# JosefAlbers/Phi-3-Vision-MLX

Measured on AMD Instinct MI355X. Metric: decode tokens/sec through generate()'s loop (reference-defined; bare graph replays: device_rate) + prefill ms, Phi-3-Vision bf16 1-image VQA, higher is better.
Workload: dtype bf16; 1 GPU; Phi-3-Vision single 336x336 image VQA (BASELINE configs[1]); 17 crops, 2509 image tokens + 22 text tokens, prompt 2531, B=1 per GPU, greedy, EOS suppressed; parallelism=batch-sharded replicas x1, batch_per_gpu=1, tiny=False

## Files before the change

### include/p3v.h

```cpp
#ifndef P3V_H
#define P3V_H
#include <stdint.h>

#ifdef __cplusplus
extern "C" {
#endif

#define P3V_VERSION 600
#define P3V_OK 0
#define P3V_ERR_ARG (-22)
#define P3V_ERR_LAUNCH (-5)
#define P3V_ERR_UNSUPPORTED (-95)
#define P3V_ERR_HIP (-14)

typedef struct {
  int cu_count, lds_per_cu, wave_size, clock_khz, mem_clock_khz, mem_bus_bits;
  int64_t hbm_bytes;
  char arch[32];
} p3v_props_t;

int p3v_version(void);
int p3v_device_props(int device, p3v_props_t* out );
const char* p3v_strerror(int code);

// ... 50 lines not shown
int p3v_gemv(const p3v_gemv_args_t* args , void* stream);

typedef struct {
  const uint16_t* x; const uint8_t* W; const float* w_scale; void* out;
  const uint16_t* resid; const uint16_t* norm_w;
  float norm_eps;
  int M, N, K;
  int epilogue;
} p3v_gemv_fp8_args_t;
int p3v_gemv_fp8(const p3v_gemv_fp8_args_t* args , void* stream);
int p3v_dequant_fp8(const uint8_t* w8, const float* w_scale, uint16_t* out_bf16, int rows, int K, void* stream);

int p3v_pack_b13(const uint16_t* W, int rows, int K, int silu_pairs, void* out, int32_t* info, void* stream);
int p3v_unpack_b13(const void* packed, int rows, int K, int silu_pairs, int exp_base, uint16_t* out_bf16, void* stream);
typedef struct {
  const uint16_t* x; const void* W; void* out;
  const uint16_t* resid; const uint16_t* norm_w;
  float norm_eps;
  int M, N, K;
  int epilogue;
  int exp_base, silu_pairs;
} p3v_gemv_b13_args_t;
int p3v_gemv_b13(const p3v_gemv_b13_args_t* args , void* stream);
int p3v_gemv_b13_plan(int N, int K, int epilogue, int n_cu, int* out );

typedef struct {
  const uint8_t* A; const float* a_scale; const uint8_t* W; const float* w_scale;
  uint16_t* out; const uint16_t* resid;
  int M, N, K, lda, ldw, ldo, epilogue;
} p3v_gemm_fp8_args_t;
int p3v_gemm_fp8(const p3v_gemm_fp8_args_t* args , void* stream);
int p3v_quant_fp8_rows(const uint16_t* x, const uint16_t* norm_w , float eps, uint8_t* q, float* scale,
                       int rows, int K, void* stream);

int p3v_rope_table(const float* pos, const float* inv_freq, float scale, float* cos_out, float* sin_out,
                   int n_pos, int half_dim, void* stream);

int p3v_rope_kv_append(const uint16_t* qkv, const float* cos_t, const float* sin_t,
                       uint16_t* q_out, uint16_t* k_dst, uint16_t* v_dst,
                       int B, int L, int n_heads, int n_kv, int hd,
                       int past, const int32_t* d_past, int dst_t, int dst_off_is_past,
                       int tab_t, int tab_div, float q_scale, void* stream);

int p3v_gemm_resid_norm(const p3v_gemm_args_t* gemm , const uint16_t* norm_w, float eps, uint16_t* normed, void* stream);

typedef struct {
  const float* cos_t; const float* sin_t;
  uint16_t* q_out; uint16_t* k_dst; uint16_t* v_dst;
  int B, L, n_heads, n_kv, hd;
  int past, dst_t, dst_off_is_past, tab_t, tab_div;
  float q_scale;
} p3v_qkv_split_t;
int p3v_gemm_qkv(const p3v_gemm_args_t* gemm , const p3v_qkv_split_t* split , void* stream);

typedef struct {
  const uint16_t* q;
  const uint16_t* k_past; const uint16_t* v_past;
  const uint16_t* k_new;  const uint16_t* v_new;
  uint16_t* out;
  const int32_t* pad_len;
  const int32_t* d_past;
  float* ws;
  int B, L, n_heads, n_kv, hd;
  int past, past_t, past_div, new_t, pad_div;
  int causal;
  float scale;
  int n_split;
  int new_is_cache;
  int q_prescaled;
} p3v_attn_args_t;
int p3v_attention(const p3v_attn_args_t* args , void* stream);
int64_t p3v_attention_ws_bytes(int B, int L, int n_heads, int hd, int n_split);
#define P3V_DECODE_MAX_L 16

typedef struct {
  const uint16_t* qkv; const float* cos_t; const float* sin_t;
  uint16_t* k_cache; uint16_t* v_cache; uint16_t* out;
  const int32_t* pad_len; const int32_t* d_past; float* ws;
  int B, L, n_heads, n_kv, hd, past, cache_t, rope_bstride, n_split;
  float scale;
  int merge_in_launch;
  const void* o_proj_w; uint16_t* o_proj_x; uint16_t* o_rearm; int o_n;
  const uint32_t* o_proj_sb;
} p3v_attn_decode_args_t;
int p3v_attention_decode(const p3v_attn_decode_args_t* args , void* stream);
int p3v_attention_decode_can_fuse_oproj(int B, int L, int n_heads, int hd, int n_split, int cache_t, int o_n, int merge_in_launch);
int p3v_attention_decode_fused_role(int wg, int n_heads, int n_split, int o_n, int map, int* out4);
#define P3V_FAMILY_MAX 16
#define P3V_FAMILY_INTS (2 + P3V_FAMILY_MAX)
int p3v_attention_decode_family(const p3v_attn_decode_args_t* args , const int32_t* family ,
                                const int32_t* family_host , void* stream);
int p3v_stage_rope(const float* cos_t, const float* sin_t, int past, const int32_t* d_past,
                   float* cos_out, float* sin_out, int B, int L, int tab_t, int half_dim, void* stream);

int p3v_kv_quantize(const uint16_t* k, const uint16_t* vt, uint8_t* k8, uint8_t* v8t, float* k_scale, float* v_scale,
                    int BH, int hd, int src_t, int dst_t, int t0, int n_tok, void* stream);
int p3v_kv_dequantize(const uint8_t* k8, const uint8_t* v8t, const float* k_scale, const float* v_scale, uint16_t* k,
                      uint16_t* vt, int BH, int hd, int src_t, int dst_t, int n_tok, void* stream);

int p3v_kv_quantize_mlx4(uint16_t* k, uint16_t* vt, uint32_t* k4, uint32_t* v4, float* k_sb, float* v_sb, int BH, int hd,
                         int cache_t, int n_tok, const uint16_t* qkv, const float* cos_t, const float* sin_t, int n_heads, int n_kv,
                         int past, int tab_t, int tab_div, void* stream);

typedef struct {
  const uint16_t* qkv; const float* cos_t; const float* sin_t;
  uint8_t* k8; uint8_t* v8t; float* k_scale; float* v_scale; uint16_t* out;
  const int32_t* pad_len; const int32_t* d_past; float* ws;
  int B, L, n_heads, n_kv, hd, past, cache_t, rope_bstride, n_split;
  float scale;
  int merge_in_launch;
  const uint8_t* o_proj_w8; const float* o_proj_scale; uint16_t* o_proj_x; uint16_t* o_rearm; int o_n;
} p3v_attn_decode_q8_args_t;
int p3v_attention_decode_q8(const p3v_attn_decode_q8_args_t* args , void* stream);
int p3v_attention_decode_q8_can_fuse_oproj(int B, int L, int n_heads, int hd, int n_split, int cache_t, int o_n, int merge_in_launch);

int p3v_im2col_patches(const float* pix, uint16_t* patches, int n_img, int img, int patch, int kpad, void* stream);
int p3v_clip_cls_rows(float* x, const uint16_t* cls, const uint16_t* pos, int n_img, int tokens, int dim, void* stream);

int p3v_hd_merge(const float* feats, const uint16_t* sub_gn, const uint16_t* glb_gn, uint16_t* out,
                 int h_crops, int w_crops, int grid , int C, void* stream);

int p3v_argmax(const uint16_t* logits, int32_t* out, int rows, int n, int64_t row_stride, void* stream);
int p3v_log_softmax(const uint16_t* x, uint16_t* y, int rows, int n, void* stream);
int p3v_topk(const uint16_t* x, int32_t* idx_out, int rows, int n, int k, int64_t row_stride, void* stream);

typedef struct {
  const uint16_t* x; const uint32_t* W; const uint32_t* sb; void* out;
  const uint16_t* resid; const uint16_t* norm_w; float norm_eps;
  int M, N, K;
  int epilogue;
} p3v_gemv_q4_args_t;
int p3v_gemv_q4(const p3v_gemv_q4_args_t* args , void* stream);
int p3v_dequant_q4(const uint32_t* w4, const uint32_t* sb, uint16_t* out_bf16, int rows, int K, void* stream);

int p3v_resample_u8(const uint8_t* in, uint8_t* out, int outer, int in_len, int out_len, int inner,
                    const int32_t* coeffs, const int32_t* bounds, int ksize, void* stream);
int p3v_hd_preprocess(const uint8_t* resized, int rh, int rw, int top, int hp, int portrait, const double* lut,
                      const float* hw, const int32_t* hi, const float* ww, const int32_t* wi, float* pixel_values,
                      int n_slots, void* stream);

int p3v_lora_down(const uint16_t* x, const float* lora_a, float* t, int M, int K, int r, void* stream);
int p3v_lora_up(const uint16_t* y, const float* t, const float* lora_b, float scale, int epilogue,
                const uint16_t* resid, uint16_t* out, int M, int N, int r, void* stream);

#define P3V_LORA_SLICE_K 256
typedef struct {
  const float* lora_a;
  const float* lora_b;
  int32_t rank;
  float scale;
} p3v_lora_entry_t;
int p3v_lora_rows_slices(int K);
int p3v_lora_down_rows(const uint16_t* x, const uint16_t* norm_w , float eps, const p3v_lora_entry_t* table,
                       const int32_t* row_adapter, float* t, int M, int K, int r_max, int n_slots, void* stream);
int p3v_lora_up_rows(const uint16_t* y, const float* t, const p3v_lora_entry_t* table, const int32_t* row_adapter,
                     int epilogue, const uint16_t* resid, uint16_t* out, int M, int N, int K, int r_max, int n_slots,
                     void* stream);

int p3v_add_i32(int32_t* x, int n, int delta, void* stream);
int p3v_store_token(const int32_t* tok, int32_t* history, const int32_t* d_step, int32_t* tok_next,
                    int B, int max_steps, void* stream);
int p3v_step_begin(const int32_t* tok, const uint16_t* table, uint16_t* x_out, const float* cos_t, const float* sin_t,
                   const int32_t* d_past, float* cos_out, float* sin_out, int B, int hidden, int vocab, int tab_t,
                   int half_dim, int32_t* zero_buf ,
                   int n_zero, void* stream);
int p3v_step_end(const uint16_t* logits, int32_t* next_tok, int32_t* tok, int32_t* history, int32_t* d_step,
// ... 115 lines not shown
```

### phi-3-vision-mlx_amd/_lib.py

```python
import ctypes as C
import os

_HERE = os.path.dirname(os.path.abspath(__file__))
LIB_PATH = os.environ.get("P3V_LIB") or os.path.join(_HERE, "libp3v.so")

P3V_OK = 0
(EPI_NONE, EPI_BIAS, EPI_BIAS_QGELU, EPI_BIAS_GELU, EPI_BIAS_RESID_F32, EPI_RESID_BF16, EPI_SILU_MUL, EPI_PATCH,
 EPI_F32) = range(9)
DECODE_MAX_L = 16

vp, i32, i64, f32 = C.c_void_p, C.c_int, C.c_int64, C.c_float


class Props(C.Structure):
    _fields_ = [("cu_count", i32), ("lds_per_cu", i32), ("wave_size", i32), ("clock_khz", i32),
                ("mem_clock_khz", i32), ("mem_bus_bits", i32), ("hbm_bytes", i64), ("arch", C.c_char * 32)]


class GemmArgs(C.Structure):
    _fields_ = [("A", vp), ("W", vp), ("out", vp), ("bias", vp), ("resid", vp), ("pos", vp),
                ("M", i32), ("N", i32), ("K", i32), ("lda", i32), ("ldw", i32), ("ldo", i32),
                ("epilogue", i32), ("patches_per_img", i32), ("ws", vp), ("ws_bytes", i64)]


class QkvSplit(C.Structure):
    _fields_ = [("cos_t", vp), ("sin_t", vp), ("q_out", vp), ("k_dst", vp), ("v_dst", vp),
                ("B", i32), ("L", i32), ("n_heads", i32), ("n_kv", i32), ("hd", i32),
                ("past", i32), ("dst_t", i32), ("dst_off_is_past", i32), ("tab_t", i32), ("tab_div", i32), ("q_scale", f32)]


class GemvArgs(C.Structure):
    _fields_ = [("x", vp), ("W", vp), ("out", vp), ("resid", vp), ("norm_w", vp), ("norm_eps", f32),
                ("M", i32), ("N", i32), ("K", i32), ("epilogue", i32)]


class GemvStep(C.Structure):
    _fields_ = [("tok", vp), ("embed_table", vp), ("vocab", i32), ("x_out", vp),
                ("cos_t", vp), ("sin_t", vp), ("cos_out", vp), ("sin_out", vp), ("tab_t", i32), ("half_dim", i32),
                ("next_tok", vp), ("tok_out", vp), ("history", vp), ("d_step", vp), ("ticket", vp), ("amax_ws", vp), ("max_steps", i32),
                ("d_past", vp)]


GEMV_STEP_WS_BYTES = 1024 * 8 + 9 * 128


class GemvF8Args(C.Structure):
    _fields_ = [("x", vp), ("W", vp), ("w_scale", vp), ("out", vp), ("resid", vp), ("norm_w", vp), ("norm_eps", f32),
                ("M", i32), ("N", i32), ("K", i32), ("epilogue", i32)]


class GemvB13Args(C.Structure):
    _fields_ = [("x", vp), ("W", vp), ("out", vp), ("resid", vp), ("norm_w", vp), ("norm_eps", f32),
                ("M", i32), ("N", i32), ("K", i32), ("epilogue", i32), ("exp_base", i32), ("silu_pairs", i32)]


class GemmF8Args(C.Structure):
    _fields_ = [("A", vp), ("a_scale", vp), ("W", vp), ("w_scale", vp), ("out", vp), ("resid", vp),
                ("M", i32), ("N", i32), ("K", i32), ("lda", i32), ("ldw", i32), ("ldo", i32), ("epilogue", i32)]


class AttnArgs(C.Structure):
    _fields_ = [("q", vp), ("k_past", vp), ("v_past", vp), ("k_new", vp), ("v_new", vp), ("out", vp),
                ("pad_len", vp), ("d_past", vp), ("ws", vp),
                ("B", i32), ("L", i32), ("n_heads", i32), ("n_kv", i32), ("hd", i32),
                ("past", i32), ("past_t", i32), ("past_div", i32), ("new_t", i32), ("pad_div", i32),
                ("causal", i32), ("scale", f32), ("n_split", i32), ("new_is_cache", i32), ("q_prescaled", i32)]


class GemvQ4Args(C.Structure):
    _fields_ = [("x", vp), ("W", vp), ("sb", vp), ("out", vp), ("resid", vp), ("norm_w", vp), ("norm_eps", f32),
                ("M", i32), ("N", i32), ("K", i32), ("epilogue", i32)]


class AttnDecArgs(C.Structure):
    _fields_ = [("qkv", vp), ("cos_t", vp), ("sin_t", vp), ("k_cache", vp), ("v_cache", vp), ("out", vp),
                ("pad_len", vp), ("d_past", vp), ("ws", vp),
                ("B", i32), ("L", i32), ("n_heads", i32), ("n_kv", i32), ("hd", i32), ("past", i32),
                ("cache_t", i32), ("rope_bstride", i32), ("n_split", i32), ("scale", f32), ("merge_in_launch", i32),
                ("o_proj_w", vp), ("o_proj_x", vp), ("o_rearm", vp), ("o_n", i32),
                ("o_proj_sb", vp)]


class AttnDecQ8Args(C.Structure):
    _fields_ = [("qkv", vp), ("cos_t", vp), ("sin_t", vp), ("k8", vp), ("v8t", vp), ("k_scale", vp), ("v_scale", vp),
                ("out", vp), ("pad_len", vp), ("d_past", vp), ("ws", vp),
                ("B", i32), ("L", i32), ("n_heads", i32), ("n_kv", i32), ("hd", i32), ("past", i32),
                ("cache_t", i32), ("rope_bstride", i32), ("n_split", i32), ("scale", f32), ("merge_in_launch", i32),
                ("o_proj_w8", vp), ("o_proj_scale", vp), ("o_proj_x", vp), ("o_rearm", vp), ("o_n", i32)]


class SampleRow(C.Structure):
    _fields_ = [("temperature", f32), ("top_k", i32), ("top_p", f32), ("seed_lo", C.c_uint32), ("seed_hi", C.c_uint32),
                ("counter", i32)]


LOGPROBS_MAX = 8


class LogprobRecord(C.Structure):
    _fields_ = [("token", C.c_int32), ("logprob", f32), ("rank", C.c_int32), ("n_top", C.c_int32),
                ("top_id", C.c_int32 * LOGPROBS_MAX), ("top_logprob", f32 * LOGPROBS_MAX)]


LOGPROB_WORDS = C.sizeof(LogprobRecord) // 4


class PenaltyRow(C.Structure):
    _fields_ = [("repetition", f32), ("frequency", f32), ("presence", f32), ("flags", C.c_int32)]


PENALTY_WORDS = C.sizeof(PenaltyRow) // 4
PENALTY_ACTIVE, PENALTY_BIAS = 1, 2


class GuideRow(C.Structure):
    _fields_ = [("flags", C.c_int32), ("n_states", C.c_int32), ("state", C.c_int32), ("reserved", C.c_int32)]


GUIDE_WORDS = C.sizeof(GuideRow) // 4
GUIDE_MAX_STATES, GUIDE_ACTIVE, GUIDE_DONE = 255, 1, -1


class KvCopyJob(C.Structure):
    _fields_ = [("k_src", vp), ("v_src", vp), ("k_dst", vp), ("v_dst", vp),
                ("ks_src", vp), ("vs_src", vp), ("ks_dst", vp), ("vs_dst", vp),
                ("B_src", i32), ("b_src", i32), ("T_src", i32), ("t0_src", i32),
                ("B_dst", i32), ("b_dst", i32), ("T_dst", i32), ("t0_dst", i32), ("n_tok", i32)]


KV_FORK_MAX_DST = 15
FAMILY_MAX, FAMILY_INTS = 16, 18


class KvFork(C.Structure):
    _fields_ = [("k_src", vp), ("v_src", vp), ("k_dst", vp), ("v_dst", vp),
                ("ks_src", vp), ("vs_src", vp), ("ks_dst", vp), ("vs_dst", vp),
                ("B_src", i32), ("b_src", i32), ("T_src", i32), ("t0_src", i32),
                ("B_dst", i32), ("T_dst", i32), ("t0_dst", i32), ("n_tok", i32), ("n_dst", i32),
                ("b_dst", i32 * KV_FORK_MAX_DST)]


class SpecState(C.Structure):
    _fields_ = [("tok", vp), ("ctx", vp), ("ctl", vp), ("amax", vp), ("ticket", vp),
                ("history", vp), ("rec", vp), ("d_step", vp), ("d_past", vp),
                ("ctx_cap", i32), ("hist_cap", i32), ("rec_cap", i32), ("n_max", i32), ("n_min", i32)]


SPEC_REC_INTS, SPEC_CTL_INTS, SPEC_NGRAM_CAP = 18, 8, 8
SPEC_CTL_N, SPEC_CTL_NDRAFT, SPEC_CTL_FORCED, SPEC_CTL_REPLAY, SPEC_CTL_NLIMIT, SPEC_CTL_ACC = range(6)
KV_COPY_MAX_JOBS = 4
LORA_SLICE_K, LORA_MAX_RANK = 256, 64
SAMPLE_MAX_N, SAMPLE_MAX_ROWS = 32768, 1024
SIGNATURES = {
    "p3v_version": (i32, []),
    "p3v_device_props": (i32, [i32, C.POINTER(Props)]),
    "p3v_strerror": (C.c_char_p, [i32]),
    "p3v_set_tuning": (i32, [C.c_char_p, i32]),
    "p3v_get_tuning": (i32, [C.c_char_p, C.POINTER(i32)]),
    "p3v_embed_gather": (i32, [vp, vp, vp, i32, i32, i32, vp]),
    "p3v_rmsnorm": (i32, [vp, vp, vp, i32, i32, f32, vp]),
    "p3v_layernorm": (i32, [vp, vp, vp, vp, i32, i32, i32, f32, vp]),
    "p3v_gemm": (i32, [C.POINTER(GemmArgs), vp]),
    "p3v_gemm_ws_bytes": (i64, [i32, i32, i32, i32]),
# ... 98 lines not shown
```

### phi-3-vision-mlx_amd/csrc/p3v_attention.hip

```cpp
#include <stdlib.h>

#include "p3v_common.h"
#include "p3v_attn_shared.h"
#include "p3v_dot_bf16.h"
#include "p3v_dot_f8.h"
#include "p3v_dot_q4.h"

struct AttnP {
  const bf16_t* q; const bf16_t* k_past; const bf16_t* v_past; const bf16_t* k_new; const bf16_t* v_new;
  bf16_t* out; const int32_t* pad_len; const int32_t* d_past; float* ws;
  int B, L, nh, nkv, past, past_t, past_div, new_t, pad_div, causal, split_mode, n_split, new_is_cache;
  float scale;
  int head_group;
  float sc2;
  int q_prescaled;
};

template <int HD>
__global__ void __launch_bounds__(256) k_attn(AttnP p) {
  constexpr int KSTR = HD * 2 + 16;
  constexpr int VSTR = 64 * 2 + 16;
  constexpr int NKS = HD / 32;
  constexpr int NDT = HD / 16;
  constexpr int CPR = HD / 8;
  __shared__ __attribute__((aligned(16))) unsigned char Ks[64 * KSTR];
  __shared__ __attribute__((aligned(16))) unsigned char Vt[HD * VSTR];

  const int tid = threadIdx.x, lane = tid & 63, wave = tid >> 6;
  const int g = lane >> 4, qi = lane & 15;
  const int b = blockIdx.z, head = blockIdx.y, kvh = head / (p.nh / p.nkv);
  const int past = p.d_past ? *p.d_past : p.past;
  const int total = past + p.L;
  const int pad = p.pad_len ? p.pad_len[b / p.pad_div] : 0;
  const float sc2 = p.sc2;

  int q0, kv_begin, kv_end;
  bool active;
  if (p.split_mode) {
    q0 = 0;
    const int chunk = ((total + p.n_split - 1) / p.n_split + 63) & ~63;
    kv_begin = blockIdx.x * chunk;
    kv_end = min(total, kv_begin + chunk);
    active = wave == 0;
  } else {
    q0 = blockIdx.x * 64 + wave * 16;
    kv_begin = 0;
    kv_end = p.causal ? min(total, past + blockIdx.x * 64 + 64) : total;
    active = q0 < p.L;
  }
  if (pad > kv_begin) kv_begin = pad & ~63;

  const int qrow = q0 + qi;
  const bool qvalid = qrow < p.L;
  bf16x8_t qf[NKS];
  {
    const bf16_t* qp = p.q + (((size_t)b * p.nh + head) * p.L + (qvalid ? qrow : 0)) * HD + 8 * g;
#pragma unroll
    for (int ks = 0; ks < NKS; ++ks) {
      u32x4_t v = *(const u32x4_t*)(qp + 32 * ks);
      if (!qvalid) v = (u32x4_t){0, 0, 0, 0};
      qf[ks] = __builtin_bit_cast(bf16x8_t, v);
    }
  }
  const int qpos = past + qrow;

  const bf16_t* kp_base = p.k_past + ((size_t)(b / p.past_div) * p.nkv + kvh) * (size_t)p.past_t * HD;
  const bf16_t* vp_base = p.v_past + ((size_t)(b / p.past_div) * p.nkv + kvh) * (size_t)HD * p.past_t;
  const bf16_t* kn_base = p.k_new + ((size_t)b * p.nkv + kvh) * (size_t)p.new_t * HD;
  const bf16_t* vn_base = p.v_new + ((size_t)b * p.nkv + kvh) * (size_t)HD * p.new_t;

  float m_run = -INFINITY, l_run = 0.f;
  f32x4_t o[NDT];
#pragma unroll
  for (int d = 0; d < NDT; ++d) o[d] = (f32x4_t){0.f, 0.f, 0.f, 0.f};

  for (int kv0 = kv_begin; kv0 < kv_end; kv0 += 64) {
    __syncthreads();
    for (int i = tid; i < 64 * CPR; i += 256) {
      const int key = i / CPR, c = i % CPR, t = kv0 + key;
      u32x4_t kv = {0, 0, 0, 0};
      if (t < kv_end) {
        const bool from_past = t < past || p.new_is_cache;
        const bf16_t* ks = from_past ? kp_base + (size_t)t * HD : kn_base + (size_t)(t - past) * HD;
        kv = *(const u32x4_t*)(ks + c * 8);
      }
      *(u32x4_t*)(Ks + key * KSTR + c * 16) = kv;
    }
    for (int i = tid; i < HD * 8; i += 256) {
      const int d = i >> 3, c = i & 7, t0 = kv0 + c * 8;
// ... 1414 lines not shown
    const float m_use = m_new == -INFINITY ? 0.f : m_new;
    float l_t = 0.f;
#pragma unroll
    for (int r = 0; r < 4; ++r) {
      s[r] = __builtin_amdgcn_exp2f(s[r] - m_use);
      l_t += s[r];
    }
    l_run = rows_sum(l_t);
    m_run = m_new;
    DBG_T(5);
    const u32x2_t pw = {pack_bf16x2(s[0], s[1]), pack_bf16x2(s[2], s[3])};
    const s16x4_t pf = __builtin_bit_cast(s16x4_t, pw);
#pragma unroll
    for (int d = 0; d < NDT; ++d) {
      const s16x4_t vf = *(const s16x4_t*)(vtile + v_rd + d * 16 * 128);
      o[d] = __builtin_amdgcn_mfma_f32_16x16x16bf16_1k(vf, pf, o[d], 0, 0, 0);
    }
    DBG_T(6);
  }

  asm volatile("s_waitcnt vmcnt(0) lgkmcnt(0)" ::: "memory");
  __syncthreads();
  if (qvalid) {
    float* Ow = (float*)wreg + qi * HD;
#pragma unroll
    for (int d = 0; d < NDT; ++d) *(f32x4_t*)(Ow + 16 * d + 4 * g) = o[d];
    if (g == 0) { Ml[wave][qi][0] = m_run; Ml[wave][qi][1] = l_run; }
  }
  __syncthreads();
#pragma unroll 1
  for (int idx = tid; idx < n_vnew; idx += 256) {
    const int q = idx / HD, d = idx - q * HD;
    float mk[4], M = -INFINITY;
#pragma unroll
    for (int k = 0; k < 4; ++k) { mk[k] = Ml[k][q][0]; M = fmaxf(M, mk[k]); }
    const float Mu = M == -INFINITY ? 0.f : M;
    float acc = 0.f, lsum = 0.f;
#pragma unroll
    for (int k = 0; k < 4; ++k) {
      const float c = __builtin_amdgcn_exp2f(mk[k] - Mu);
      acc += c * ((const float*)(KV + k * WREG))[q * HD + d];
      lsum += c * Ml[k][q][1];
    }
    float* w = p.ws + ((((size_t)b * p.nh + head) * p.n_split + bx) * 16 + q) * (HD + 2);
    st_wt(w + d, acc);
    if (d == 0) { st_wt(w + HD, M); st_wt(w + HD + 1, lsum); }
  }
  DBG_T(7);
  DBG_W(13, false);
  if (p.merge && bx == p.n_split - 1) {
    __shared__ float merge_scratch[SPLIT_MERGE_SCRATCH(256)];
    split_merge<256>(p.ws + ((size_t)b * p.nh + head) * p.n_split * 16 * (HD + 2), p.out + (size_t)b * p.L * (p.nh * HD) + head * HD,
                     (size_t)p.nh * HD, p.L, p.n_split, nullptr, merge_scratch);
  }
  DBG_W(11, false);
}

struct FoMap { int bx, by, o_unit, o_unit2; };
__host__ __device__ __forceinline__ bool fo_map_ok(int n_split, int nh, int o_n) { return nh == 32 && o_n == 3072 && n_split >= 13 && n_split * nh <= 768; }
__host__ __device__ __forceinline__ FoMap fo_map(int L, int n_split, int nh, int n_units, bool two_on_last) {
  const int G = n_split * nh, base = G >> 8, r = G & 255;
  const int v = L & 255, slot = L >> 8, ns = base + (v < r ? 1 : 0);
  const int m0 = (base - 1) * 256 + 224;
  FoMap m;
  m.o_unit = m.o_unit2 = -1;
  if (L >= m0 && L < m0 + 32) { m.by = L - m0; m.bx = n_split - 1; return m; }
  const int before = L - m0 < 0 ? 0 : (L - m0 > 32 ? 32 : L - m0);
  const int u = L - before;
  m.by = u / (n_split - 1);
  m.bx = u - m.by * (n_split - 1);
  if (v < 224) {
    const int from_last = ns - 1 - slot;
    const int idx = base >= 2 || two_on_last ? (v >= r ? v - r : (224 - r) + v) : v;
    const int second = 224 + idx < n_units ? 224 + idx : -1;
    if (from_last == 0) { m.o_unit = v; if (two_on_last) m.o_unit2 = second; }
    else if (from_last == 1 && !two_on_last) m.o_unit = second;
  }
  return m;
}

#ifndef P3V_FO_SLEEP
#define P3V_FO_SLEEP 4
#endif
enum { FO_NONE = 0, FO_BF16 = 1, FO_F8 = 2, FO_Q4 = 3 };
struct FoP { const void* o_w; const void* o_scale; bf16_t* o_x; const bf16_t* out; int nh; };
template <int KIND, int NU = 1>
__device__ __forceinline__ void fo_project(const FoP f, const int o_wl, unsigned char* lds, const int o_wl2 = -1) {
  constexpr bool F8 = KIND == FO_F8, Q4 = KIND == FO_Q4;
  constexpr int HD = 96, NJ = KIND == FO_BF16 ? 6 : 3;
  const int tid = threadIdx.x, lane = tid & 63, wave = __builtin_amdgcn_readfirstlane(tid >> 6);
  const int Kd = f.nh * HD;
  const size_t row_bytes = (size_t)Kd * (Q4 ? 1 : F8 ? 2 : 4) / 2;
  const bool two = NU > 1 && o_wl2 >= 0;
  int o_u[NU];
  u32x4_t ow[NU][2][Q4 ? 1 : NJ];
  u32x2_t oq[NU][2][Q4 ? 3 : 1];
  uint32_t osb[NU][2][Q4 ? 3 : 1];
  uint32_t ores[NU];
  float osc[NU][2];
#pragma unroll
  for (int k = 0; k < NU; ++k) {
    o_u[k] = (k == 0 ? o_wl : o_wl2) * 4 + wave;
    if (k == 1 && !two) continue;
    const unsigned char* r0p = (const unsigned char*)f.o_w + (size_t)(2 * o_u[k]) * row_bytes;
    if (Q4) {
      const uint32_t* s0 = (const uint32_t*)f.o_scale + (size_t)(2 * o_u[k]) * (Kd / 64) + (lane >> 2);
#pragma unroll
      for (int j = 0; j < 3; ++j) {
        oq[k][0][j] = __builtin_nontemporal_load((const u32x2_t*)r0p + j * 64 + lane);
        oq[k][1][j] = __builtin_nontemporal_load((const u32x2_t*)(r0p + row_bytes) + j * 64 + lane);
        osb[k][0][j] = s0[j * 16];
        osb[k][1][j] = s0[Kd / 64 + j * 16];
      }
    } else {
#pragma unroll
      for (int j = 0; j < NJ; ++j) {
        ow[k][0][j] = __builtin_nontemporal_load((const u32x4_t*)r0p + j * 64 + lane);
        ow[k][1][j] = __builtin_nontemporal_load((const u32x4_t*)(r0p + row_bytes) + j * 64 + lane);
      }
    }
    ores[k] = *(const uint32_t*)(f.o_x + 2 * o_u[k]);
    osc[k][0] = F8 ? ((const float*)f.o_scale)[2 * o_u[k]] : 1.f;
    osc[k][1] = F8 ? ((const float*)f.o_scale)[2 * o_u[k] + 1] : 1.f;
  }
  {
    __shared__ int o_timeout;
    const uint32_t* src = (const uint32_t*)f.out;
    if (wave == 0) {
      bool to = false;
      const long long t_wait = wall_clock64();
      for (unsigned tries = 0;; ++tries) {
        const uint32_t c = lane < f.nh ? __hip_atomic_load(src + lane * (HD / 2) + HD / 2 - 1, __ATOMIC_RELAXED, __HIP_MEMORY_SCOPE_AGENT) : 0u;
        if (!__any((c & 0xffffu) == 0xffffu || (c >> 16) == 0xffffu)) break;
        if ((tries & 15u) == 15u && wall_clock64() - t_wait > 500000) { to = true; break; }
        __builtin_amdgcn_s_sleep(P3V_FO_SLEEP);
      }
      if (lane == 0) o_timeout = to;
    }
    TMARK(12);
    __syncthreads();
    uint32_t* xs = (uint32_t*)lds;
    bool timeout = o_timeout != 0;
    {
      const int NW = f.nh * HD / 2 / 4;
      uint32_t xv[6];
      for (unsigned tries = 0; !timeout; ++tries) {
        bool bad = false;
#pragma unroll
        for (int j = 0; j < 6; ++j) xv[j] = __hip_atomic_load(src + wave * NW + j * 64 + lane, __ATOMIC_RELAXED, __HIP_MEMORY_SCOPE_AGENT);
#pragma unroll
        for (int j = 0; j < 6; ++j) bad |= (xv[j] & 0xffffu) == 0xffffu || (xv[j] >> 16) == 0xffffu;
        if (!__any(bad)) break;
        if (tries >= (1u << 12)) timeout = true;
        __builtin_amdgcn_s_sleep(2);
      }
#pragma unroll
      for (int j = 0; j < 6; ++j) xs[wave * NW + j * 64 + lane] = xv[j];
      if (timeout && lane == 0) o_timeout = 1;
    }
    __syncthreads();
    timeout = o_timeout != 0;
    float* xsum = (float*)(lds + 6144);
    if (Q4) {
      if (tid < 192) {
        const u32x4_t a = ((const u32x4_t*)xs)[2 * tid], b = ((const u32x4_t*)xs)[2 * tid + 1];
        float t = 0.f;
#pragma unroll
        for (int j = 0; j < 4; ++j) t += (bf16lo(a[j]) + bf16hi(a[j])) + (bf16lo(b[j]) + bf16hi(b[j]));
        xsum[tid] = t;
      }
      __syncthreads();
    }
#pragma unroll
    for (int k = 0; k < NU; ++k) {
      if (k == 1 && !two) continue;
      float a0 = 0.f, a1 = 0.f;
      if (Q4) {
#pragma unroll
        for (int j = 0; j < 3; ++j) {
          const int pc = j * 64 + lane;
          const u32x4_t xa = ((const u32x4_t*)xs)[2 * pc], xb = ((const u32x4_t*)xs)[2 * pc + 1];
          const float X = xsum[pc], X128 = 128.f * X;
#pragma unroll
          for (int h = 0; h < 2; ++h) {
            const float D = dot8_q4(oq[k][h][j][1], xb, dot8_q4(oq[k][h][j][0], xa, 0.f));
            const float c = bf16lo(osb[k][h][j]) * (D - X128) + bf16hi(osb[k][h][j]) * X;
            if (h == 0) a0 += c; else a1 += c;
          }
        }
        if (k == 0) TMARK(13);
        a0 = wave_sum(a0);
        a1 = wave_sum(a1);
      } else if (F8) {
#pragma unroll
        for (int j = 0; j < 3; ++j) {
          const u32x4_t xa = ((const u32x4_t*)xs)[2 * (j * 64 + lane)], xb = ((const u32x4_t*)xs)[2 * (j * 64 + lane) + 1];
          a0 = dot16_f8(ow[k][0][j], xa, xb, a0);
          a1 = dot16_f8(ow[k][1][j], xa, xb, a1);
        }
        if (k == 0) TMARK(13);
        a0 = wave_sum(a0) * osc[k][0];
        a1 = wave_sum(a1) * osc[k][1];
      } else {
#pragma unroll
        for (int j = 0; j < 6; ++j) {
          const u32x4_t xa = ((const u32x4_t*)xs)[j * 64 + lane];
          a0 = dot8(ow[k][0][j], xa, a0);
          a1 = dot8(ow[k][1][j], xa, a1);
        }
        if (k == 0) TMARK(13);
        a0 = wave_sum(a0);
        a1 = wave_sum(a1);
      }
      if (lane == 0) {
        const float v0 = bf16lo(ores[k]) + bf16_round(a0), v1 = bf16hi(ores[k]) + bf16_round(a1);
        *(uint32_t*)(f.o_x + 2 * o_u[k]) = timeout ? 0x7fc07fc0u : pack_bf16x2(v0, v1);
      }
    }
    TMARK(14);
  }
}

template <int FO = 0>
__device__ __forceinline__ void attn_decode_body128(const AttnDecP& p, const int bx, const int by, const int bz, unsigned char* KV,
                                                    const int o_unit = -2, const int o_unit2 = -1) {
  constexpr int TK = 128, WK = 32, HD = 96, KROW = HD * 2, VROWB = TK * 2, NKS = 3, NDT = 6, CPR = 12;
  constexpr int KS_BYTES = WK * KROW;
  static_assert(KS_BYTES >= 16 * HD * 4, "a wave's O partial reuses its K slice");
  __shared__ __attribute__((aligned(16))) unsigned char Qs[16 * KROW];
  __shared__ float Ml[4][16][2];
  const int tid = threadIdx.x, lane = tid & 63, g = lane >> 4, qi = lane & 15;
  const int wave = __builtin_amdgcn_readfirstlane(tid >> 6);
  const int b = bz, head = by, kvh = (head * p.grp_magic) >> 16;
  const bool kv_writer = head == kvh * p.grp;
  unsigned char* kslice = KV + wave * KS_BYTES;
  unsigned char* vtile = KV + 4 * KS_BYTES;

  TMARK(0);
#ifdef P3V_ATTN_TIMING
  {
    unsigned hw, xcc;
    asm volatile("s_getreg_b32 %0, hwreg(HW_REG_HW_ID)" : "=s"(hw));
    asm volatile("s_getreg_b32 %0, hwreg(HW_REG_XCC_ID)" : "=s"(xcc));
    TVAL(15, (long long)(((xcc & 15) << 8) | (((hw >> 13) & 7) << 5) | (((hw >> 12) & 1) << 4) | ((hw >> 8) & 15)));
  }
#endif
  int past = p.past, pad = 0;
  const int past_lb = p.past;
  if (p.d_past) asm volatile("s_load_dword %0, %1, 0x0" : "=s"(past) : "s"(p.d_past) : "memory");
  if (p.pad_len) asm volatile("s_load_dword %0, %1, 0x0" : "=s"(pad) : "s"(p.pad_len + b) : "memory");

  const unsigned char* kc = (const unsigned char*)(p.k_cache + ((size_t)b * p.nkv + kvh) * (size_t)p.cache_t * HD);
  bf16_t* vc = p.v_cache + ((size_t)b * p.nkv + kvh) * (size_t)HD * p.cache_t;
  const int kv_lo = bx * TK, kv_hi = min(p.cache_t, kv_lo + TK);
  const size_t vrow = (size_t)p.cache_t * 2;
  auto issue_dma = [&]() {
    const int kv0 = min(kv_lo, p.cache_t - TK);
    const unsigned char* ksrc = kc + (size_t)(kv0 + WK * wave) * KROW;
    const unsigned char* vs = (const unsigned char*)vc + (size_t)kv0 * 2;
    const __amdgpu_buffer_rsrc_t rs_k = __builtin_amdgcn_make_buffer_rsrc((void*)ksrc, 0, 0xffffffff, 0x00020000);
    const __amdgpu_buffer_rsrc_t rs_v = __builtin_amdgcn_make_buffer_rsrc((void*)vs, 0, 0xffffffff, 0x00020000);
#pragma unroll
    for (int j = 0; j < 6; ++j) {
      const int i = j * 64 + lane, r0 = i / CPR, pc = i - r0 * CPR;
      const unsigned koff = r0 * KROW + ((pc ^ ((r0 >> 2) & 3)) << 4);
      __builtin_amdgcn_raw_ptr_buffer_load_lds(rs_k, (dec_lptr_t)(kslice + j * 1024), 16, koff, 0, 0, P3V_ATTN_AUX);
    }
#pragma unroll
    for (int j = 0; j < 6; ++j) {
      const int d = 24 * wave + 4 * j + (lane >> 4);
      const unsigned voff = (unsigned)d * (unsigned)vrow + ((((unsigned)lane & 15) ^ ((unsigned)d & 15)) << 4);
      __builtin_amdgcn_raw_ptr_buffer_load_lds(rs_v, (dec_lptr_t)(vtile + wave * 6144 + j * 1024), 16, voff, 0, 0, P3V_ATTN_AUX);
    }
  };

  const int row_w = (p.nh + 2 * p.nkv) * HD;
  const float* cos_b = p.cos_t + (size_t)b * p.rope_bstride * (HD / 2);
  const float* sin_b = p.sin_t + (size_t)b * p.rope_bstride * (HD / 2);
  const int tr = tid / CPR, tc = tid - tr * CPR;
  const bool rtask = tr < p.L;
  RopeRaw qraw, kraw;
  if (rtask) {
    const bf16_t* row = p.qkv + ((size_t)b * p.L + tr) * row_w;
    qraw = rope_fetch(row + head * HD, tc, cos_b + tr * (HD / 2), sin_b + tr * (HD / 2));
    const bf16_t* krow = row + (p.nh + kvh) * HD;
    kraw = qraw;
    kraw.x0 = *(const u32x4_t*)(krow + tc * 8);
    kraw.x1 = *(const u32x4_t*)(krow + (tc < 6 ? tc * 8 + 48 : tc * 8 - 48));
  }
  const bf16_t* vnew = p.qkv + (size_t)b * p.L * row_w + (p.nh + p.nkv + kvh) * HD;
  const int n_vnew = p.L * HD;
  bf16_t v_early = 0;
  if (tid < n_vnew) {
    const int r = tid / HD;
    v_early = vnew[(size_t)r * row_w + (tid - r * HD)];
  }
  const bool surely_live = p.d_past ? (past_lb < 0 || bx * TK < past_lb) : bx * TK < past_lb + p.L;
  if (surely_live) issue_dma();
  TMARK(7);
  const unsigned qs_lds = (unsigned)(size_t)(dec_lptr_t)Qs;
  if (tid < 16 * CPR) {
    u32x4_t v = {0, 0, 0, 0};
    if (rtask) v = rope_apply(qraw, tc);
    asm volatile("ds_write_b128 %0, %1" ::"v"(qs_lds + tr * KROW + ((tc ^ ((tr >> 2) & 3)) << 4)), "v"(v) : "memory");
  }

  asm volatile("s_waitcnt lgkmcnt(0)" : "+s"(past), "+s"(pad)::"memory");
  const int total = past + p.L;
// ... 90 lines not shown
        const int t = kv0 + WK * wave + 16 * kb + 4 * g + r;
        const bool vis = t < kv_end && t >= pad && t <= qpos && qpos >= pad;
        s[kb][r] = vis ? s[kb][r] * sc2 : -INFINITY;
        m_t = fmaxf(m_t, s[kb][r]);
      }
    m_t = rows_max(m_t);
    const float m_use = m_t == -INFINITY ? 0.f : m_t;
    float l_t = 0.f;
#pragma unroll
    for (int kb = 0; kb < 2; ++kb)
#pragma unroll
      for (int r = 0; r < 4; ++r) {
        s[kb][r] = __builtin_amdgcn_exp2f(s[kb][r] - m_use);
        l_t += s[kb][r];
      }
    l_run = rows_sum(l_t);
    m_run = m_t;
    if (l_run == 12345.f) TVAL(15, 1);
    TMARK(10);
    const u32x4_t pw = {pack_bf16x2(s[0][0], s[0][1]), pack_bf16x2(s[0][2], s[0][3]), pack_bf16x2(s[1][0], s[1][1]), pack_bf16x2(s[1][2], s[1][3])};
    const bf16x8_t pf = __builtin_bit_cast(bf16x8_t, pw);
    if (!has_new) {
      asm volatile("s_waitcnt vmcnt(0)\n\ts_barrier" ::: "memory");
    }
#pragma unroll
    for (int d = 0; d < NDT; ++d) {
      const u32x2_t a0 = *(const u32x2_t*)(vtile + v_rd[0] + d * 16 * VROWB), a1 = *(const u32x2_t*)(vtile + v_rd[1] + d * 16 * VROWB);
      const u32x4_t aw = {a0[0], a0[1], a1[0], a1[1]};
      o[d] = __builtin_amdgcn_mfma_f32_16x16x32_bf16(__builtin_bit_cast(bf16x8_t, aw), pf, o[d], 0, 0, 0);
    }
  }

  const bool merger = p.merge && bx == p.n_split - 1;
  float* own = (float*)(vtile + 4096);
  static_assert(SPLIT_MERGE_SCRATCH(256) * 4 <= 4096 && 4096 + 16 * (HD + 2) * 4 <= 96 * 256, "merge scratch + own partial fit the V^T tile");
  if (o[0][0] == 12345.f) TVAL(15, 2);
  TMARK(11);
  asm volatile("s_waitcnt vmcnt(0) lgkmcnt(0)" ::: "memory");
  __syncthreads();
  TMARK(2);
  const int o_wl = o_unit != -2 ? o_unit : by * (p.n_split - 1) + bx;
  const bool o_worker = FO && !merger && bx < p.n_split - 1 && o_wl >= 0 && o_wl * 8 < p.o_n;
  if (FO) {
    if (bx == 0 && by == 0) {
      uint32_t* ra = (uint32_t*)p.o_rearm;
      for (int i = tid; i < p.nh * HD / 2; i += 256) ra[i] = 0xffffffffu;
    }
  }
  if (qvalid) {
    float* Ow = (float*)kslice + qi * HD;
#pragma unroll
    for (int d = 0; d < NDT; ++d) *(f32x4_t*)(Ow + 16 * d + 4 * g) = o[d];
    if (g == 0) { Ml[wave][qi][0] = m_run; Ml[wave][qi][1] = l_run; }
  }
  __syncthreads();
#pragma unroll 1
  for (int idx = tid; idx < n_vnew; idx += 256) {
    const int q = idx / HD, d = idx - q * HD;
    float mk[4], M = -INFINITY;
#pragma unroll
    for (int k = 0; k < 4; ++k) { mk[k] = Ml[k][q][0]; M = fmaxf(M, mk[k]); }
    const float Mu = M == -INFINITY ? 0.f : M;
    float acc = 0.f, lsum = 0.f;
#pragma unroll
    for (int k = 0; k < 4; ++k) {
      const float c = __builtin_amdgcn_exp2f(mk[k] - Mu);
      acc += c * ((const float*)(KV + k * KS_BYTES))[q * HD + d];
      lsum += c * Ml[k][q][1];
    }
    if (merger) {
      own[q * (HD + 2) + d] = acc;
      if (d == 0) { own[q * (HD + 2) + HD] = M; own[q * (HD + 2) + HD + 1] = lsum; }
    } else {
      float* w = p.ws + ((((size_t)b * p.nh + head) * p.n_split + bx) * 16 + q) * (HD + 2);
      st_wt(w + d, acc);
      if (d == 0) { st_wt(w + HD, M); st_wt(w + HD + 1, lsum); }
    }
  }
  TMARK(3);
  if (merger)
    split_merge<256>(p.ws + ((size_t)b * p.nh + head) * p.n_split * 16 * (HD + 2), p.out + (size_t)b * p.L * (p.nh * HD) + head * HD,
                     (size_t)p.nh * HD, p.L, p.n_split, own, (float*)vtile, FO != 0);
  if (FO && o_worker) {
    fo_project<FO, 2>(FoP{p.o_w, p.o_sb, p.o_x, p.out, p.nh}, o_wl, KV, o_unit2);
  }
}

__global__ void __launch_bounds__(256) k_attn_decode128(AttnDecP p) {
  __shared__ __attribute__((aligned(1024))) unsigned char KV[4 * 6144 + 96 * 256];
  attn_decode_body128<FO_NONE>(p, blockIdx.x, blockIdx.y, blockIdx.z, KV);
}

__global__ void __launch_bounds__(256) k_attn_decode128_o(AttnDecP p) {
  __shared__ __attribute__((aligned(1024))) unsigned char KV[4 * 6144 + 96 * 256];
  int bx = blockIdx.x, by = blockIdx.y, o_unit = -2, o_unit2 = -1;
  if (p.fo_remap) {
    const FoMap m = fo_map((int)blockIdx.x, p.n_split, p.nh, p.o_n / 8, p.fo_remap == 2);
    bx = m.bx, by = m.by, o_unit = m.o_unit, o_unit2 = m.o_unit2;
  }
  attn_decode_body128<FO_BF16>(p, bx, by, blockIdx.z, KV, o_unit, o_unit2);
}

__global__ void __launch_bounds__(256) k_attn_decode128_o4(AttnDecP p) {
  __shared__ __attribute__((aligned(1024))) unsigned char KV[4 * 6144 + 96 * 256];
  int bx = blockIdx.x, by = blockIdx.y, o_unit = -2, o_unit2 = -1;
  if (p.fo_remap) {
    const FoMap m = fo_map((int)blockIdx.x, p.n_split, p.nh, p.o_n / 8, p.fo_remap == 2);
    bx = m.bx, by = m.by, o_unit = m.o_unit, o_unit2 = m.o_unit2;
  }
  attn_decode_body128<FO_Q4>(p, bx, by, blockIdx.z, KV, o_unit, o_unit2);
}

__global__ void __launch_bounds__(256) k_attn_decode(AttnDecP p) {
  __shared__ __attribute__((aligned(1024))) unsigned char KV[4 * 6144];
  attn_decode_body(p, blockIdx.x, blockIdx.y, blockIdx.z, KV);
}

template <int TK>
__global__ void __launch_bounds__(64) k_attn_decode_stream(AttnDecP p) {
  constexpr int HD = 96, KSTR = HD * 2 + 16, VSTR = TK * 2 + 16, NKS = 3, NDT = 6, CPR = 12;
  constexpr int KIT = TK * CPR / 64, VCH = TK / 8, VIT = HD * VCH / 64;
  __shared__ __attribute__((aligned(16))) unsigned char Ks[TK * KSTR];
  __shared__ __attribute__((aligned(16))) unsigned char Vt[HD * VSTR];
  const int lane = threadIdx.x, g = lane >> 4, qi = lane & 15;
  const int b = blockIdx.z, head = blockIdx.y, kvh = (head * p.grp_magic) >> 16;
  const bool kv_writer = head == kvh * p.grp;
  const float sc2 = p.scale * 1.4426950408889634f;
  const int row_w = (p.nh + 2 * p.nkv) * HD;
  const bf16_t* kc = p.k_cache + ((size_t)b * p.nkv + kvh) * (size_t)p.cache_t * HD;
  bf16_t* vc = p.v_cache + ((size_t)b * p.nkv + kvh) * (size_t)HD * p.cache_t;
  const int chunk = p.chunk;
  const int kv_lo = blockIdx.x * chunk, kv_hi = min(p.cache_t, kv_lo + chunk);

  u32x4_t kreg[KIT], vreg[VIT];
  auto load_tile = [&](int kv0) {
#pragma unroll
    for (int it = 0; it < KIT; ++it) {
      const int i = it * 64 + lane;
      kreg[it] = __builtin_nontemporal_load((const u32x4_t*)(kc + (size_t)(kv0 + i / CPR) * HD + (i % CPR) * 8));
    }
#pragma unroll
    for (int it = 0; it < VIT; ++it) {
      const int i = it * 64 + lane;
      vreg[it] = __builtin_nontemporal_load((const u32x4_t*)(vc + (size_t)(i / VCH) * p.cache_t + kv0 + (i % VCH) * 8));
    }
  };
  if (kv_lo < kv_hi) load_tile(kv_lo);

  const int past = p.d_past ? *p.d_past : p.past;
  const int total = past + p.L;
  const int pad = p.pad_len ? p.pad_len[b] : 0;
  int kv_begin = kv_lo;
  const int kv_end = min(total, kv_hi);
  if (pad > kv_begin) kv_begin = pad & ~(TK - 1);
  const float* cos_b = p.cos_t + (size_t)b * p.rope_bstride * (HD / 2);
  const float* sin_b = p.sin_t + (size_t)b * p.rope_bstride * (HD / 2);

  auto patch_new = [&](int kv0) {
    const int n0 = max(past, kv0), n1 = min(kv_end, kv0 + TK), n_new = n1 - n0;
#pragma unroll 1
    for (int w = lane; w < n_new * CPR; w += 64) {
      const int t = n0 + w / CPR, c = w % CPR, r = t - past;
      const bf16_t* row = p.qkv + ((size_t)b * p.L + r) * row_w;
      const u32x4_t kn = rope_chunk(row + (p.nh + kvh) * HD, c, cos_b + r * (HD / 2), sin_b + r * (HD / 2));
      *(u32x4_t*)(Ks + (t - kv0) * KSTR + c * 16) = kn;
      if (kv_writer) *(u32x4_t*)(p.k_cache + (((size_t)b * p.nkv + kvh) * p.cache_t + t) * HD + c * 8) = kn;
    }
#pragma unroll 1
    for (int w = lane; w < n_new * HD; w += 64) {
      const int t = n0 + w / HD, d = w % HD, r = t - past;
      const bf16_t val = p.qkv[((size_t)b * p.L + r) * row_w + (p.nh + p.nkv + kvh) * HD + d];
      *(bf16_t*)(Vt + d * VSTR + (t - kv0) * 2) = val;
      if (kv_writer) vc[(size_t)d * p.cache_t + t] = val;
    }
  };
  if (kv_begin > kv_lo && kv_begin < kv_end) load_tile(kv_begin);


  const bool qvalid = qi < p.L;
  const int qpos = past + qi;
  bf16x8_t qf[NKS];
  {
    const bf16_t* qrow = p.qkv + ((size_t)b * p.L + (qvalid ? qi : 0)) * row_w + head * HD;
    const float* ct = cos_b + (qvalid ? qi : 0) * (HD / 2);
    const float* st = sin_b + (qvalid ? qi : 0) * (HD / 2);
#pragma unroll
    for (int ks = 0; ks < NKS; ++ks) {
      u32x4_t v = rope_chunk(qrow, 4 * ks + g, ct, st);
      if (!qvalid) v = (u32x4_t){0, 0, 0, 0};
      qf[ks] = __builtin_bit_cast(bf16x8_t, v);
    }
  }

// ... 91 lines not shown
                    (size_t)p.nh * HD, p.L, p.n_split, nullptr, merge_scratch);
  }
}

template <bool WT>
__device__ __forceinline__ void combine_rows(const float* __restrict__ ws, bf16_t* __restrict__ out, int L, int nh, int hd, int n_split, int block) {
  __shared__ float pm[CMB_G], pl[CMB_G];
  __shared__ float part[CMB_G][128];
  const int qi = block % L, head = (block / L) % nh, b = block / (L * nh);
  const float* base = ws + (((size_t)b * nh + head) * n_split * 16 + qi) * (hd + 2);
  const size_t sstr = (size_t)16 * (hd + 2);
  const int t = threadIdx.x, grp = t >> 6, d0 = t & 63;
  const int G = blockDim.x >> 6;
  const int per = (n_split + G - 1) / G, s0 = grp * per, s1 = min(n_split, s0 + per);
  const bool two = d0 + 64 < hd;
  float m = -INFINITY, l = 0.f, a0 = 0.f, a1 = 0.f;
#pragma unroll 4
  for (int s = s0; s < s1; ++s) {
    const float ms = base[s * sstr + hd], ls = base[s * sstr + hd + 1];
    const float o0 = base[s * sstr + d0], o1 = two ? base[s * sstr + d0 + 64] : 0.f;
    const float mn = fmaxf(m, ms);
    const float mu = mn == -INFINITY ? 0.f : mn;
    const float ca = __builtin_amdgcn_exp2f(m - mu), cb = __builtin_amdgcn_exp2f(ms - mu);
    l = l * ca + ls * cb;
    a0 = a0 * ca + o0 * cb;
    a1 = a1 * ca + o1 * cb;
    m = mn;
  }
  {
    float* wbase = const_cast<float*>(base);
    const float sentinel = __builtin_bit_cast(float, WS_SENTINEL);
    for (int s = s0; s < s1; ++s) {
      wbase[s * sstr + d0] = sentinel;
      if (two) wbase[s * sstr + d0 + 64] = sentinel;
      if (d0 == 0) { wbase[s * sstr + hd] = sentinel; wbase[s * sstr + hd + 1] = sentinel; }
    }
  }
  if (d0 == 0) { pm[grp] = m; pl[grp] = l; }
  part[grp][d0] = a0;
  if (two) part[grp][d0 + 64] = a1;
  __syncthreads();
  auto elem = [&](int e) {
    float M = pm[0];
    for (int k = 1; k < G; ++k) M = fmaxf(M, pm[k]);
    const float Mu = M == -INFINITY ? 0.f : M;
    float acc = 0.f, lsum = 0.f;
#pragma unroll 4
    for (int k = 0; k < G; ++k) {
      const float c = __builtin_amdgcn_exp2f(pm[k] - Mu);
      acc += c * part[k][e];
      lsum += c * pl[k];
    }
    return lsum > 0.f ? acc / lsum : 0.f;
  };
  bf16_t* row = out + ((size_t)b * L + qi) * (size_t)(nh * hd) + head * hd;
  if (WT) {
    if (t < hd / 2) __hip_atomic_store((uint32_t*)row + t, pack_bf16x2(elem(2 * t), elem(2 * t + 1)), __ATOMIC_RELAXED, __HIP_MEMORY_SCOPE_AGENT);
  } else if (t < hd) {
    row[t] = f32_to_bf16(elem(t));
  }
}

__global__ void __launch_bounds__(64 * CMB_G) k_attn_combine2(const float* __restrict__ ws, bf16_t* __restrict__ out, int L,
                                                              int nh, int hd, int n_split) {
  combine_rows<false>(ws, out, L, nh, hd, n_split, (int)blockIdx.x);
}

template <int KIND>
__global__ void __launch_bounds__(512) k_attn_combine_o(const float* __restrict__ ws, bf16_t* __restrict__ out, bf16_t* __restrict__ o_rearm,
                                                        const void* o_w, const void* o_sb, bf16_t* o_x, int nh, int n_split, int n_units) {
  __shared__ __attribute__((aligned(16))) unsigned char lds[7 * 1024 + 768];
  if ((int)blockIdx.x < nh) {
    if (blockIdx.x == 0) {
      uint32_t* ra = (uint32_t*)o_rearm;
      for (int i = threadIdx.x; i < nh * 96 / 2; i += blockDim.x) ra[i] = 0xffffffffu;
    }
    combine_rows<true>(ws, out, 1, nh, 96, n_split, (int)blockIdx.x);
    return;
  }
  if (threadIdx.x >= 256) return;
  const int n_uw = (int)gridDim.x - nh, u = (int)blockIdx.x - nh;
  fo_project<KIND, 2>(FoP{o_w, o_sb, o_x, out, nh}, u, lds, u + n_uw < n_units ? u + n_uw : -1);
}

static bool combine_o_ok(int B, int L, int n_heads, int hd, int n_split, int o_n) {
  if (B != 1 || L != 1 || hd != 96 || n_heads * hd != 3072 || o_n <= 0 || o_n % 8) return false;
  if (n_split < 1 || n_split > 128 || combine_threads(n_split) > 512) return false;
  int dev = 0;
  hipDeviceProp_t pr;
  if (hipGetDevice(&dev) != hipSuccess || hipGetDeviceProperties(&pr, dev) != hipSuccess) return false;
  return n_heads + (o_n / 8 + 1) / 2 <= pr.multiProcessorCount - 8;
}
template <int KIND>
static int launch_combine_o(const float* ws, void* out, void* o_rearm, const void* o_w, const void* o_sb, void* o_x, int n_heads, int n_split,
                            int o_n, hipStream_t s) {
  const int n_units = o_n / 8, grid_o = n_heads + (n_units + 1) / 2;
  hipLaunchKernelGGL(k_attn_combine_o<KIND>, dim3(grid_o), dim3(combine_threads(n_split)), 0, s, ws, (bf16_t*)out, (bf16_t*)o_rearm, o_w, o_sb,
                     (bf16_t*)o_x, n_heads, n_split, n_units);
  P3V_CHECK_LAUNCH();
  return P3V_OK;
}

__global__ void k_stage_rope(const float* __restrict__ cos_t, const float* __restrict__ sin_t, const int32_t* d_past,
                             int past, float* __restrict__ cos_o, float* __restrict__ sin_o, int L, int tab_t, int half) {
  if (d_past) past = *d_past;
  const int b = blockIdx.x / L, r = blockIdx.x % L;
  for (int i = threadIdx.x; i < half; i += blockDim.x) {
    cos_o[((size_t)b * L + r) * half + i] = cos_t[((size_t)b * tab_t + past + r) * half + i];
    sin_o[((size_t)b * L + r) * half + i] = sin_t[((size_t)b * tab_t + past + r) * half + i];
  }
}

extern "C" int p3v_stage_rope(const float* cos_t, const float* sin_t, int past, const int32_t* d_past, float* cos_out,
                              float* sin_out, int B, int L, int tab_t, int half_dim, void* stream) {
  if (!cos_t || !sin_t || !cos_out || !sin_out || B <= 0 || L <= 0) return P3V_ERR_ARG;
  hipLaunchKernelGGL(k_stage_rope, dim3(B * L), dim3(64), 0, (hipStream_t)stream, cos_t, sin_t, d_past, past, cos_out,
                     sin_out, L, tab_t, half_dim);
  P3V_CHECK_LAUNCH();
  return P3V_OK;
}

#ifdef P3V_ATTN_DEBUG
extern "C" int p3v_debug_read(unsigned long long* out) {
  return hipMemcpyFromSymbol(out, HIP_SYMBOL(p3v_dbg), sizeof(unsigned long long) * 16) == hipSuccess ? 0 : -1;
}
#endif

extern "C" int p3v_attention_decode_can_fuse_oproj(int B, int L, int n_heads, int hd, int n_split, int cache_t, int o_n, int merge_in_launch) {
  if (B != 1 || L != 1 || hd != 96 || n_heads * hd != 3072 || o_n <= 0 || o_n % 8) return 0;
  if (!merge_in_launch)
    return combine_o_ok(B, L, n_heads, hd, n_split, o_n) ? 2 : 0;
  if (!(n_split * 128 >= cache_t && cache_t % 128 == 0 && n_split * 64 < cache_t) || n_split < 2) return 0;
  if ((long)(n_split - 1) * n_heads * 8 < o_n) return 0;
  static long capacity_of[P3V_MAX_DEVICES] = {0};
  int dev = 0;
  if (hipGetDevice(&dev) != hipSuccess || dev < 0 || dev >= P3V_MAX_DEVICES) return 0;
  if (!capacity_of[dev]) {
    int per_cu = 0;
    hipDeviceProp_t pr;
    if (hipGetDeviceProperties(&pr, dev) != hipSuccess) return 0;
    int per_cu4 = 0;
    if (hipOccupancyMaxActiveBlocksPerMultiprocessor(&per_cu, k_attn_decode128_o, 256, 0) != hipSuccess ||
        hipOccupancyMaxActiveBlocksPerMultiprocessor(&per_cu4, k_attn_decode128_o4, 256, 0) != hipSuccess) return 0;
    per_cu = min(per_cu, per_cu4);
    if (per_cu < 1) return 0;
    capacity_of[dev] = (long)per_cu * (pr.multiProcessorCount - 8);
  }
  const long capacity = capacity_of[dev];
  return (long)B * n_heads * n_split <= capacity;
}

extern "C" int p3v_attention_decode_fused_role(int wg, int n_heads, int n_split, int o_n, int map, int* out4) {
  if (!out4 || wg < 0 || n_split < 2 || n_heads < 1 || wg >= n_heads * n_split || (map != 1 && map != 2)) return P3V_ERR_ARG;
  if (!fo_map_ok(n_split, n_heads, o_n)) return P3V_ERR_UNSUPPORTED;
  const FoMap m = fo_map(wg, n_split, n_heads, o_n / 8, map == 2);
  out4[0] = m.bx, out4[1] = m.by, out4[2] = m.o_unit, out4[3] = m.o_unit2;
  return P3V_OK;
}

extern "C" int p3v_attention_decode(const p3v_attn_decode_args_t* a, void* stream) {
  if (!a || !a->qkv || !a->cos_t || !a->sin_t || !a->k_cache || !a->v_cache || !a->out || !a->ws) return P3V_ERR_ARG;
  if (a->hd != 96) return P3V_ERR_UNSUPPORTED;
  if (a->B <= 0 || a->L <= 0 || a->L > P3V_DECODE_MAX_L || a->n_heads % a->n_kv) return P3V_ERR_ARG;
  if (a->n_split < 1 || a->n_split > 128 || a->cache_t % 64) return P3V_ERR_ARG;
  if (((uintptr_t)a->ws | (uintptr_t)a->out) & 15) return P3V_ERR_ARG;
  const int grp = a->n_heads / a->n_kv;
  const int chunk = ((a->cache_t + a->n_split - 1) / a->n_split + 63) & ~63;
  AttnDecP p = {a->qkv, a->cos_t, a->sin_t, a->k_cache, a->v_cache, a->pad_len, a->d_past, a->ws,
                a->B, a->L, a->n_heads, a->n_kv, a->past, a->cache_t, a->rope_bstride, a->n_split, a->scale,
                chunk, grp, (65536 + grp - 1) / grp, a->merge_in_launch, (bf16_t*)a->out,
                a->o_proj_w, a->o_proj_sb, (bf16_t*)a->o_proj_x, (bf16_t*)a->o_rearm, a->o_n, 0};
  hipStream_t s = (hipStream_t)stream;
  dim3 grid(a->n_split, a->n_heads, a->B);
  const int fuse_form = a->o_proj_w ? p3v_attention_decode_can_fuse_oproj(a->B, a->L, a->n_heads, a->hd, a->n_split, a->cache_t, a->o_n, a->merge_in_launch) : 0;
  if (a->o_proj_w && !fuse_form) return P3V_ERR_UNSUPPORTED;
  if (a->o_proj_w && (!a->o_proj_x || !a->o_rearm || ((uintptr_t)a->o_proj_w | (uintptr_t)a->o_proj_x | (uintptr_t)a->o_rearm) & 15)) return P3V_ERR_ARG;
  if (a->o_proj_w && a->o_proj_sb && ((uintptr_t)a->o_proj_sb & 3)) return P3V_ERR_ARG;
  if (fuse_form == 1) {
    if (p3v_tuning().attn_fo_map && fo_map_ok(a->n_split, a->n_heads, a->o_n)) {
      p.fo_remap = p3v_tuning().attn_fo_map;
      grid = dim3(a->n_split * a->n_heads, 1, 1);
    }
    if (a->o_proj_sb) {
      if ((uintptr_t)a->o_proj_sb & 3) return P3V_ERR_ARG;
      hipLaunchKernelGGL(k_attn_decode128_o4, grid, dim3(256), 0, s, p);
    } else {
      hipLaunchKernelGGL(k_attn_decode128_o, grid, dim3(256), 0, s, p);
    }
    P3V_CHECK_LAUNCH();
    return P3V_OK;
  }
  if (a->n_split * 64 >= a->cache_t) hipLaunchKernelGGL(k_attn_decode, grid, dim3(256), 0, s, p);
  else if (a->n_split * 128 >= a->cache_t && a->cache_t % 128 == 0) hipLaunchKernelGGL(k_attn_decode128, grid, dim3(256), 0, s, p);
  else hipLaunchKernelGGL(k_attn_decode_stream<64>, grid, dim3(64), 0, s, p);
  P3V_CHECK_LAUNCH();
  if (a->merge_in_launch) return P3V_OK;
  if (fuse_form == 2)
    return a->o_proj_sb ? launch_combine_o<FO_Q4>(a->ws, a->out, a->o_rearm, a->o_proj_w, a->o_proj_sb, a->o_proj_x, a->n_heads, a->n_split, a->o_n, s)
                        : launch_combine_o<FO_BF16>(a->ws, a->out, a->o_rearm, a->o_proj_w, nullptr, a->o_proj_x, a->n_heads, a->n_split, a->o_n, s);
  hipLaunchKernelGGL(k_attn_combine2, dim3(a->B * a->n_heads * a->L), dim3(combine_threads(a->n_split)), 0, s, a->ws, a->out, a->L, a->n_heads,
                     a->hd, a->n_split);
  P3V_CHECK_LAUNCH();
  return P3V_OK;
}

__global__ void __launch_bounds__(256) k_kv_quantize(const bf16_t* __restrict__ k, const bf16_t* __restrict__ vt,
                                                     uint8_t* __restrict__ k8, uint8_t* __restrict__ v8,
                                                     float* __restrict__ ksc, float* __restrict__ vsc, int hd, int src_t,
                                                     int dst_t, int t0, int n_tok) {
  __shared__ float vmax[64];
  __shared__ bf16_t vtile[96 * 66];
  const int bh = blockIdx.y, tt = blockIdx.x * 64, tid = threadIdx.x, lane = tid & 63, wave = tid >> 6;
  for (int r = wave; r < 64; r += 4) {
    const int t = t0 + tt + r;
    if (tt + r >= n_tok) break;
    const bf16_t* row = k + ((size_t)bh * src_t + t) * hd;
    const float a = lane < hd / 2 ? bf16_to_f32(row[2 * lane]) : 0.f, b = lane < hd / 2 ? bf16_to_f32(row[2 * lane + 1]) : 0.f;
    const float amax = wave_max(fmaxf(fabsf(a), fabsf(b)));
    const float s = amax > 0.f ? amax / 127.f : 1.f, inv = 1.f / s;
    if (lane < hd / 2) {
      const int qa = (int)rintf(a * inv) + 128, qb = (int)rintf(b * inv) + 128;
      *(uint16_t*)(k8 + ((size_t)bh * dst_t + t) * hd + 2 * lane) = (uint16_t)(qa | (qb << 8));
    }
    if (lane == 0) ksc[(size_t)bh * dst_t + t] = s;
  }
  for (int i = tid; i < hd * 64; i += 256) {
    const int d = i >> 6, c = i & 63;
    vtile[d * 66 + c] = tt + c < n_tok ? vt[((size_t)bh * hd + d) * src_t + t0 + tt + c] : (bf16_t)0;
  }
  __syncthreads();
  if (tid < 64) {
    float m = 0.f;
    for (int d = 0; d < hd; ++d) m = fmaxf(m, fabsf(bf16_to_f32(vtile[d * 66 + tid])));
    vmax[tid] = m > 0.f ? m / 127.f : 1.f;
    if (tt + tid < n_tok) vsc[(size_t)bh * dst_t + t0 + tt + tid] = vmax[tid];
  }
  __syncthreads();
  for (int i = tid; i < hd * 64; i += 256) {
    const int d = i >> 6, c = i & 63;
    if (tt + c < n_tok)
      v8[((size_t)bh * hd + d) * dst_t + t0 + tt + c] = (uint8_t)((int)rintf(bf16_to_f32(vtile[d * 66 + c]) / vmax[c]) + 128);
  }
}

__global__ void __launch_bounds__(256) k_kv_quantize_v(const bf16_t* __restrict__ k, const bf16_t* __restrict__ vt,
                                                       uint8_t* __restrict__ k8, uint8_t* __restrict__ v8,
                                                       float* __restrict__ ksc, float* __restrict__ vsc, int src_t, int dst_t,
                                                       int t0, int n_tok) {
  constexpr int HD = 96;
  __shared__ unsigned vmax_bits[64];
  const int bh = blockIdx.y, tt = blockIdx.x * 64, tid = threadIdx.x, lane = tid & 63;
  if (tid < 64) vmax_bits[tid] = 0u;
  u32x4_t vv[3];
#pragma unroll
  for (int j = 0; j < 3; ++j) {
    const int i = j * 256 + tid, d = i >> 3, c = i & 7;
    vv[j] = *(const u32x4_t*)(vt + ((size_t)bh * HD + d) * src_t + t0 + tt + 8 * c);
  }
#pragma unroll
  for (int pass = 0; pass < 4; ++pass) {
    const int r = pass * 16 + (tid >> 4), c = tid & 15, t = t0 + tt + r;
    const bool live = c < 12 && tt + r < n_tok;
    u32x4_t w = {0u, 0u, 0u, 0u};
    if (live) w = *(const u32x4_t*)(k + ((size_t)bh * src_t + t) * HD + c * 8);
    float amax = 0.f;
#pragma unroll
    for (int j = 0; j < 4; ++j) amax = fmaxf(amax, fmaxf(fabsf(bf16lo(w[j])), fabsf(bf16hi(w[j]))));
    amax = fmaxf(amax, P3V_DPP_F32(amax, 0xB1));
    amax = fmaxf(amax, P3V_DPP_F32(amax, 0x4E));
    amax = fmaxf(amax, P3V_DPP_F32(amax, 0x124));
    amax = fmaxf(amax, P3V_DPP_F32(amax, 0x128));
    const float sc = amax > 0.f ? amax / 127.f : 1.f, inv = 1.f / sc;
    if (live) {
      u32x2_t o;
#pragma unroll
      for (int h = 0; h < 2; ++h) {
        const int q0 = (int)rintf(bf16lo(w[2 * h]) * inv) + 128, q1 = (int)rintf(bf16hi(w[2 * h]) * inv) + 128;
        const int q2 = (int)rintf(bf16lo(w[2 * h + 1]) * inv) + 128, q3 = (int)rintf(bf16hi(w[2 * h + 1]) * inv) + 128;
        o[h] = (uint32_t)q0 | ((uint32_t)q1 << 8) | ((uint32_t)q2 << 16) | ((uint32_t)q3 << 24);
// ... 880 lines not shown
```

### phi-3-vision-mlx_amd/csrc/p3v_common.h

```cpp
#pragma once
#include <hip/hip_runtime.h>
#include <stdint.h>

#include "../../include/p3v.h"

typedef uint16_t bf16_t;
typedef __attribute__((ext_vector_type(8))) __bf16 bf16x8_t;
typedef __attribute__((ext_vector_type(4))) float f32x4_t;
typedef __attribute__((ext_vector_type(16))) float f32x16_t;
typedef __attribute__((ext_vector_type(4))) uint32_t u32x4_t;
typedef __attribute__((ext_vector_type(2))) uint32_t u32x2_t;

#define P3V_WAVE 64
#define P3V_MAX_DEVICES 64

#define P3V_CHECK_LAUNCH()                                   \
  do {                                                       \
    hipError_t e_ = hipGetLastError();                       \
    if (e_ != hipSuccess) return P3V_ERR_LAUNCH;             \
  } while (0)

__device__ __forceinline__ float bf16_to_f32(bf16_t u) { return __uint_as_float(((uint32_t)u) << 16); }

typedef __attribute__((ext_vector_type(2))) __bf16 bf16x2_t;
// ... 27 lines not shown
__device__ __forceinline__ void rows_swap32(float v, float& a, float& b) {
  const unsigned u = __builtin_bit_cast(unsigned, v);
  auto r = __builtin_amdgcn_permlane32_swap(u, u, false, false);
  unsigned x = r[0], y = r[1];
  asm("" : "+v"(x), "+v"(y));
  a = __builtin_bit_cast(float, x); b = __builtin_bit_cast(float, y);
}
__device__ __forceinline__ void rows_swap16(float v, float& a, float& b) {
  const unsigned u = __builtin_bit_cast(unsigned, v);
  auto r = __builtin_amdgcn_permlane16_swap(u, u, false, false);
  unsigned x = r[0], y = r[1];
  asm("" : "+v"(x), "+v"(y));
  a = __builtin_bit_cast(float, x); b = __builtin_bit_cast(float, y);
}
__device__ __forceinline__ float rows_max(float v) {
  float a, b;
  rows_swap32(v, a, b); v = fmaxf(a, b);
  rows_swap16(v, a, b); return fmaxf(a, b);
}
__device__ __forceinline__ float rows_sum(float v) {
  float a, b;
  rows_swap32(v, a, b); v = a + b;
  rows_swap16(v, a, b); return a + b;
}

#define P3V_DPP_F32(v, ctrl) __builtin_bit_cast(float, __builtin_amdgcn_update_dpp(0, __builtin_bit_cast(int, v), ctrl, 0xf, 0xf, true))
__device__ __forceinline__ float wave_sum(float v) {
  v += P3V_DPP_F32(v, 0xB1);
  v += P3V_DPP_F32(v, 0x4E);
  v += P3V_DPP_F32(v, 0x124);
  v += P3V_DPP_F32(v, 0x128);
  return rows_sum(v);
}
__device__ __forceinline__ float wave_max(float v) {
  v = fmaxf(v, P3V_DPP_F32(v, 0xB1));
  v = fmaxf(v, P3V_DPP_F32(v, 0x4E));
  v = fmaxf(v, P3V_DPP_F32(v, 0x124));
  v = fmaxf(v, P3V_DPP_F32(v, 0x128));
  return rows_max(v);
}

__device__ __forceinline__ float block_sum(float v, float* red) {
  v = wave_sum(v);
  const int w = threadIdx.x >> 6, nw = blockDim.x >> 6;
  __syncthreads();
  if ((threadIdx.x & 63) == 0) red[w] = v;
  __syncthreads();
  float t = 0.f;
  for (int i = 0; i < nw; ++i) t += red[i];
  return t;
}
__device__ __forceinline__ float block_max(float v, float* red) {
  v = wave_max(v);
  const int w = threadIdx.x >> 6, nw = blockDim.x >> 6;
  __syncthreads();
  if ((threadIdx.x & 63) == 0) red[w] = v;
  __syncthreads();
  float t = -INFINITY;
  for (int i = 0; i < nw; ++i) t = fmaxf(t, red[i]);
  return t;
}

static inline int p3v_cdiv(long a, long b) { return (int)((a + b - 1) / b); }
static inline int p3v_gemv_wpw(int waves, int n_cu, int forced) {
  if (forced == 3 || forced == 4) return forced;
  const float w3 = (float)p3v_cdiv(p3v_cdiv(waves, 3), n_cu) * 3.f * n_cu / (float)waves;
  const float w4 = (float)p3v_cdiv(p3v_cdiv(waves, 4), n_cu) * 4.f * n_cu / (float)waves;
  return w3 < w4 - 0.05f ? 3 : 4;
}

struct P3vTuning {
  int gemm_big_rows;
  int gemm_no_splitk, gemm_splitk_max_m, gemm_splitk_max_s, gemm_splitk_wgs, gemm_128, gemm_persistent;
  int gemm_rows;
  int gemm_no_skinny, gemm_skinny_max_m, gemm_skinny_s, gemm_skinny_tm128;
  int gemm_no_qkv_fuse;
  int gemm_f8_narrow;
  int attn_no_dma, attn_old, attn_pp, attn_il, attn_il_waves, combine_g, kvq_old, q8_old;
  int attn_fo_map_q8;
  int attn_fo_map;
  int gemv_no_mfma, gemv_no_mfma8, gemv_wpc, gemv8_wgs, gemv_variant, gemv_rows, gemv8_min, gemv_mfma8, gemv_f8_wpc, gemv_q4_wpc, gemv_wpw, gemv_q4_rows_wgs, gemv_q4_rows8;
  int gemv_b13_wpc, gemv_b13_wpc_end;
  int gemv_b13_xscale;
};
const P3vTuning& p3v_tuning();
```

### phi-3-vision-mlx_amd/csrc/p3v_dot_b13.h

```cpp
#pragma once
#include "p3v_common.h"

template <int CH> struct B13 {
  static_assert(CH == 4 || CH == 6, "a container is 26 or 39 dwords per lane");
  static constexpr int D = 13 * CH / 2, NS = D - 6 * CH;
  static constexpr int NIB_OFF = 64 * NS, LO_OFF = NIB_OFF + (CH / 2) * 256, DWORDS = 64 * D;
  static __host__ __device__ constexpr int sign_word(int row, int j, int half) { return (row * 2 * CH + 2 * j + half) >> 3; }
  static __host__ __device__ constexpr int sign_shift(int row, int j, int half) { return (row * 2 * CH + 2 * j + half) & 7; }
};

typedef unsigned short b13_u16x2_t __attribute__((ext_vector_type(2)));

__device__ __forceinline__ void b13_pre8(uint32_t lo0, uint32_t lo1, uint32_t nib, uint32_t sg0, uint32_t sg1, uint32_t (&pre)[4]) {
  const uint32_t hi0 = (sg0 & 0x80808080u) | (nib & 0x0f0f0f0fu), hi1 = (sg1 & 0x80808080u) | ((nib >> 4) & 0x0f0f0f0fu);
  pre[0] = __builtin_amdgcn_perm(hi0, lo0, 0x05010400u);
  pre[1] = __builtin_amdgcn_perm(hi0, lo0, 0x07030602u);
  pre[2] = __builtin_amdgcn_perm(hi1, lo1, 0x05010400u);
  pre[3] = __builtin_amdgcn_perm(hi1, lo1, 0x07030602u);
}

__device__ __forceinline__ u32x4_t b13_decode8(uint32_t lo0, uint32_t lo1, uint32_t nib, uint32_t sg0, uint32_t sg1, uint32_t cc) {
  uint32_t pre[4];
  b13_pre8(lo0, lo1, nib, sg0, sg1, pre);
  const b13_u16x2_t c2 = __builtin_bit_cast(b13_u16x2_t, cc), one = {1, 1}, mag = {0x7fff, 0x7fff};
  u32x4_t w;
#pragma unroll
  for (int d = 0; d < 4; ++d) {
    const b13_u16x2_t p = __builtin_bit_cast(b13_u16x2_t, pre[d]);
    b13_u16x2_t n, r;
    asm("v_pk_min_u16 %0, %1, %2" : "=v"(n) : "v"(p & mag), "v"(one));
    asm("v_pk_mad_u16 %0, %1, %2, %3" : "=v"(r) : "v"(n), "v"(c2), "v"(p));
    w[d] = __builtin_bit_cast(uint32_t, r);
  }
  return w;
}
```

### phi-3-vision-mlx_amd/csrc/p3v_gemv_b13.hip

```cpp
#include <type_traits>

#include "p3v_common.h"
#include "p3v_dot_b13.h"
#include "p3v_dot_bf16.h"
#include "p3v_gemv3_body.h"

struct GemvB13P {
  const bf16_t* x; const uint32_t* W; void* out; const bf16_t* resid; const bf16_t* norm_w;
  float eps;
  int M, N, K, epi, units;
  uint32_t cc;
};

#ifdef P3V_GEMV_TIMING
__device__ long long p3v_gemv_b13_tbuf[4096 * 3];
extern "C" int p3v_gemv_b13_timing_read(long long* out, int n) {
  return hipMemcpyFromSymbol(out, HIP_SYMBOL(p3v_gemv_b13_tbuf), sizeof(long long) * n) == hipSuccess ? 0 : -1;
}
#define B13MARK(k) do { if ((threadIdx.x & 63) == 0 && blockIdx.x < 1024) p3v_gemv_b13_tbuf[(blockIdx.x * 4 + (threadIdx.x >> 6)) * 3 + (k)] = wall_clock64(); } while (0)
#else
#define B13MARK(k)
#endif
template <int CH, bool WITH_CC> struct B13Stage { uint32_t sg[B13<CH>::NS]; u32x4_t nib[CH / 2]; u32x4_t lo[CH]; uint32_t cc; };
template <int CH> struct B13Stage<CH, false> { uint32_t sg[B13<CH>::NS]; u32x4_t nib[CH / 2]; u32x4_t lo[CH]; };
template <bool SCALED> struct GemvB13 {
  typedef GemvB13P P;
  static constexpr int WPL = 8, MAX_MT = 1, MIN_WG = 4;
  static constexpr bool XSUM = false, XSCALE = SCALED;
  template <int CH> using Stage = B13Stage<CH, !SCALED>;
  static int wpc() { return p3v_tuning().gemv_b13_wpc; }
  static int wpc_end() { return p3v_tuning().gemv_b13_wpc_end; }
  static __device__ __forceinline__ void mark(int k) { B13MARK(k); }
  template <int K, int CH>
  static __device__ __forceinline__ void load(const P& p, int r0, int, int c0, Stage<CH>& st) {
    typedef B13<CH> L;
    constexpr int NST = K / (CH * 512);
    const int u = p.epi == P3V_EPI_SILU_MUL ? r0 : r0 >> 1, lane = c0 & 63, s = (c0 >> 6) / CH;
    const uint32_t* cp = p.W + (size_t)(u * NST + s) * L::DWORDS;
    if constexpr (L::NS == 3) {
      const uint32_t* sp = cp + lane * 3;
      st.sg[0] = __builtin_nontemporal_load(sp);
      st.sg[1] = __builtin_nontemporal_load(sp + 1);
      st.sg[2] = __builtin_nontemporal_load(sp + 2);
    } else {
      const u32x2_t v = __builtin_nontemporal_load((const u32x2_t*)cp + lane);
      st.sg[0] = v[0];
      st.sg[1] = v[1];
    }
    const u32x4_t* np = (const u32x4_t*)(cp + L::NIB_OFF) + lane;
    const u32x4_t* lp = (const u32x4_t*)(cp + L::LO_OFF) + lane;
#pragma unroll
    for (int i = 0; i < CH / 2; ++i) st.nib[i] = __builtin_nontemporal_load(np + i * 64);
#pragma unroll
    for (int j = 0; j < CH; ++j) st.lo[j] = __builtin_nontemporal_load(lp + j * 64);
    if constexpr (!SCALED) st.cc = p.cc;
  }
  template <bool EXACT, int CH>
  static __device__ __forceinline__ u32x4_t weights_as(const Stage<CH>& st, uint32_t cc, int j, int row) {
    typedef B13<CH> L;
    const uint32_t lo0 = st.lo[j][2 * row], lo1 = st.lo[j][2 * row + 1], nib = st.nib[j >> 1][(j & 1) * 2 + row];
    const uint32_t sg0 = st.sg[L::sign_word(row, j, 0)] << L::sign_shift(row, j, 0), sg1 = st.sg[L::sign_word(row, j, 1)] << L::sign_shift(row, j, 1);
    if constexpr (EXACT) return b13_decode8(lo0, lo1, nib, sg0, sg1, cc);
    else {
      uint32_t pre[4];
      b13_pre8(lo0, lo1, nib, sg0, sg1, pre);
      return (u32x4_t){pre[0], pre[1], pre[2], pre[3]};
    }
  }
  template <int CH>
  static __device__ __forceinline__ u32x4_t weights(const Stage<CH>& st, int j, int row) {
    static_assert(!SCALED, "the bf16 weights: the exact form only");
    return weights_as<true>(st, st.cc, j, row);
  }
  template <int CH>
  static __device__ __forceinline__ void dot(const Stage<CH>& st, int j, const u32x4_t* x, const float*, int c, float& a0, float& a1) {
    const u32x4_t xa = x[c];
    if constexpr (SCALED) {
      a0 = dot8(weights_as<false>(st, 0u, j, 0), xa, a0);
      a1 = dot8(weights_as<false>(st, 0u, j, 1), xa, a1);
    } else {
      a0 = dot8(weights(st, j, 0), xa, a0);
      a1 = dot8(weights(st, j, 1), xa, a1);
    }
  }
  template <int CH>
  static __device__ __forceinline__ void dot_exact(const P& p, const Stage<CH>& st, int j, const u32x4_t* x, const float*, int c, float& a0, float& a1) {
    const u32x4_t xa = x[c];
    a0 = dot8(weights_as<true>(st, p.cc, j, 0), xa, a0);
    a1 = dot8(weights_as<true>(st, p.cc, j, 1), xa, a1);
  }
  static __device__ __forceinline__ uint32_t stage_x(const P& p, uint32_t x2, uint32_t (&acc)[2]) {
    const b13_u16x2_t one = {1, 1};
    const uint32_t mag = x2 & 0x7fff7fffu;
    uint32_t nz, y2, m1;
    asm("v_pk_min_u16 %0, %1, %2" : "=v"(nz) : "v"(mag), "v"(one));
    asm("v_pk_mad_u16 %0, %1, %2, %3" : "=v"(y2) : "v"(nz), "v"(p.cc), "v"(x2));
    asm("v_pk_max_u16 %0, %1, %2" : "=v"(acc[0]) : "v"(acc[0]), "v"(mag));
    asm("v_pk_sub_u16 %0, %1, %2" : "=v"(m1) : "v"(mag), "v"(one));
    asm("v_pk_min_u16 %0, %1, %2" : "=v"(acc[1]) : "v"(acc[1]), "v"(m1));
    return y2;
  }
  static __device__ __forceinline__ bool x_unfit(const P& p, const uint32_t (&acc)[2]) {
    const uint32_t top = 0x7f80u - (p.cc & 0xffffu);
    const uint32_t mx = max(acc[0] & 0xffffu, acc[0] >> 16), mn = min(acc[1] & 0xffffu, acc[1] >> 16);
    return mx >= top || mn < 0x7fu;
  }
  template <int CH> static __device__ __forceinline__ float finish(float v, const Stage<CH>&, int) { return v; }
};

#define B13_BAD_VALUE 1
#define B13_BAD_RANGE 2

__global__ void k_b13_init(int32_t* info) { info[0] = 0; info[1] = 1; info[2] = 255; info[3] = 0; }

__global__ void __launch_bounds__(256) k_b13_range(const u32x4_t* __restrict__ W, long chunks, int32_t* info) {
  int emin = 255, emax = 0, bad = 0;
  for (long i = (long)blockIdx.x * 256 + threadIdx.x; i < chunks; i += (long)gridDim.x * 256) {
    const u32x4_t w = W[i];
#pragma unroll
    for (int k = 0; k < 8; ++k) {
      const uint32_t h = (w[k >> 1] >> (16 * (k & 1))) & 0xffffu, e = (h >> 7) & 0xffu, m = h & 0x7fu;
      if (e == 255u || (e == 0u && m != 0u)) bad = 1;
      if (e != 0u) { emin = min(emin, (int)e); emax = max(emax, (int)e); }
    }
  }
#pragma unroll
  for (int off = 32; off > 0; off >>= 1) {
    emin = min(emin, __shfl_xor(emin, off, 64));
    emax = max(emax, __shfl_xor(emax, off, 64));
    bad |= __shfl_xor(bad, off, 64);
  }
  if ((threadIdx.x & 63) == 0) {
    atomicMin(info + 2, emin);
    atomicMax(info + 3, emax);
    if (bad) atomicOr(info, B13_BAD_VALUE);
  }
}

template <int CH>
__global__ void __launch_bounds__(256) k_b13_pack(const u32x4_t* __restrict__ W, uint32_t* __restrict__ out, int32_t* info, int rows, int nst,
                                                  int silu_pairs, long n_lanes) {
  typedef B13<CH> L;
  const int emin = info[2], emax = info[3];
  const int base = max(1, emax - 30);
  const long t = (long)blockIdx.x * 256 + threadIdx.x;
  if (t == 0) {
    info[1] = base;
    if (emin < base) atomicOr(info, B13_BAD_RANGE);
  }
  if (t >= n_lanes || emin < base) return;
  const long ci = t >> 6;
  const int lane = (int)(t & 63), u = (int)(ci / nst), s = (int)(ci % nst), xch = nst * CH * 64;
  const int r[2] = {silu_pairs ? u : 2 * u, silu_pairs ? u + rows / 2 : 2 * u + 1};
  uint32_t sg[L::NS] = {};
  u32x4_t nib[CH / 2], lo[CH];
#pragma unroll
  for (int i = 0; i < CH / 2; ++i) nib[i] = (u32x4_t){0, 0, 0, 0};
#pragma unroll
  for (int j = 0; j < CH; ++j) lo[j] = (u32x4_t){0, 0, 0, 0};
#pragma unroll
  for (int row = 0; row < 2; ++row)
#pragma unroll
    for (int j = 0; j < CH; ++j) {
      const u32x4_t w = W[(size_t)r[row] * xch + (s * CH + j) * 64 + lane];
#pragma unroll
      for (int k = 0; k < 8; ++k) {
        const uint32_t h = (w[k >> 1] >> (16 * (k & 1))) & 0xffffu, e = (h >> 7) & 0xffu, m = h & 0x7fu, sign = h >> 15;
        const uint32_t q = e == 0u ? 0u : (e - (uint32_t)base + 1u) & 31u;
        const int half = k >> 2, b = k & 3;
        lo[j][2 * row + half] |= (((q & 1u) << 7) | m) << (8 * b);
        nib[j >> 1][(j & 1) * 2 + row] |= (q >> 1) << (4 * (2 * b + half));
        sg[L::sign_word(row, j, half)] |= sign << (8 * b + 7 - L::sign_shift(row, j, half));
      }
    }
  uint32_t* cp = out + (size_t)ci * L::DWORDS;
#pragma unroll
  for (int i = 0; i < L::NS; ++i) cp[lane * L::NS + i] = sg[i];
#pragma unroll
  for (int i = 0; i < CH / 2; ++i) ((u32x4_t*)(cp + L::NIB_OFF))[i * 64 + lane] = nib[i];
#pragma unroll
  for (int j = 0; j < CH; ++j) ((u32x4_t*)(cp + L::LO_OFF))[j * 64 + lane] = lo[j];
}

template <int K, int CH>
__global__ void __launch_bounds__(256) k_b13_unpack(GemvB13P p, u32x4_t* __restrict__ out, int rows, long n_lanes) {
  constexpr int NST = K / (CH * 512);
  const long t = (long)blockIdx.x * 256 + threadIdx.x;
  if (t >= n_lanes) return;
  const long ci = t >> 6;
  const int lane = (int)(t & 63), u = (int)(ci / NST), s = (int)(ci % NST);
  const bool silu = p.epi == P3V_EPI_SILU_MUL;
  const int r[2] = {silu ? u : 2 * u, silu ? u + rows / 2 : 2 * u + 1};
  GemvB13<false>::Stage<CH> st;
  GemvB13<false>::load<K, CH>(p, r[0], r[1], s * CH * 64 + lane, st);
#pragma unroll
  for (int row = 0; row < 2; ++row)
#pragma unroll
    for (int j = 0; j < CH; ++j) out[(size_t)r[row] * (K / 8) + (s * CH + j) * 64 + lane] = GemvB13<false>::weights(st, j, row);
}

static bool b13_shape_ok(int rows, int K) { return rows > 0 && rows % 2 == 0 && (K == 3072 || K == 8192); }
static uint32_t b13_cc(int base) { const uint32_t c = (uint32_t)(base - 1) << 7; return c | (c << 16); }

extern "C" int p3v_pack_b13(const uint16_t* W, int rows, int K, int silu_pairs, void* out, int32_t* info, void* stream) {
  if (!W || !out || !info) return P3V_ERR_ARG;
  if (!b13_shape_ok(rows, K)) return P3V_ERR_UNSUPPORTED;
  if (((uintptr_t)W | (uintptr_t)out) & 15) return P3V_ERR_ARG;
  hipStream_t s = (hipStream_t)stream;
  const long chunks = (long)rows * (K / 8), n_lanes = chunks / (K == 3072 ? 12 : 8);
  hipLaunchKernelGGL(k_b13_init, dim3(1), dim3(1), 0, s, info);
  hipLaunchKernelGGL(k_b13_range, dim3(min(4096, p3v_cdiv(chunks, 256))), dim3(256), 0, s, (const u32x4_t*)W, chunks, info);
  if (K == 3072) hipLaunchKernelGGL(k_b13_pack<6>, dim3(p3v_cdiv(n_lanes, 256)), dim3(256), 0, s, (const u32x4_t*)W, (uint32_t*)out, info, rows, 1, silu_pairs, n_lanes);
  else hipLaunchKernelGGL(k_b13_pack<4>, dim3(p3v_cdiv(n_lanes, 256)), dim3(256), 0, s, (const u32x4_t*)W, (uint32_t*)out, info, rows, 4, silu_pairs, n_lanes);
  P3V_CHECK_LAUNCH();
  return P3V_OK;
}

extern "C" int p3v_unpack_b13(const void* packed, int rows, int K, int silu_pairs, int exp_base, uint16_t* out, void* stream) {
  if (!packed || !out || exp_base < 1 || exp_base > 224) return P3V_ERR_ARG;
  if (!b13_shape_ok(rows, K)) return P3V_ERR_UNSUPPORTED;
  if (((uintptr_t)packed | (uintptr_t)out) & 15) return P3V_ERR_ARG;
  GemvB13P p = {nullptr, (const uint32_t*)packed, nullptr, nullptr, nullptr, 0.f, 1, rows, K, silu_pairs ? P3V_EPI_SILU_MUL : P3V_EPI_NONE, rows / 2, b13_cc(exp_base)};
  const long n_lanes = (long)rows * (K / 8) / (K == 3072 ? 12 : 8);
  hipStream_t s = (hipStream_t)stream;
  if (K == 3072) hipLaunchKernelGGL((k_b13_unpack<3072, 6>), dim3(p3v_cdiv(n_lanes, 256)), dim3(256), 0, s, p, (u32x4_t*)out, rows, n_lanes);
  else hipLaunchKernelGGL((k_b13_unpack<8192, 4>), dim3(p3v_cdiv(n_lanes, 256)), dim3(256), 0, s, p, (u32x4_t*)out, rows, n_lanes);
  P3V_CHECK_LAUNCH();
  return P3V_OK;
}

#define B13_XSCALE_MAX_SHIFT 96
static int b13_params(const p3v_gemv_b13_args_t* a, GemvB13P& p, bool& scaled) {
  if (a->M <= 0 || a->N <= 0) return P3V_ERR_ARG;
  if (a->M != 1 || a->N % 2 || (a->K != 3072 && a->K != 8192)) return P3V_ERR_UNSUPPORTED;
  if (a->exp_base < 1 || a->exp_base > 224 || ((uintptr_t)a->W & 15)) return P3V_ERR_ARG;
  if ((a->silu_pairs != 0) != (a->epilogue == P3V_EPI_SILU_MUL)) return P3V_ERR_ARG;
  scaled = p3v_tuning().gemv_b13_xscale != 0 && a->exp_base - 1 <= B13_XSCALE_MAX_SHIFT && a->K == 3072;
  p = {a->x, (const uint32_t*)a->W, a->out, a->resid, a->norm_w, a->norm_eps, a->M, a->N, a->K, a->epilogue,
       a->epilogue == P3V_EPI_SILU_MUL ? a->N : a->N / 2, b13_cc(a->exp_base)};
  return P3V_OK;
}

extern "C" int p3v_gemv_b13_plan(int N, int K, int epilogue, int n_cu, int* out) {
  if (!out || N <= 0 || n_cu <= 0) return P3V_ERR_ARG;
  if (N % 2 || (K != 3072 && K != 8192)) return P3V_ERR_UNSUPPORTED;
  const GemvPlan g = gemv_stream_plan(epilogue == P3V_EPI_SILU_MUL ? N : N / 2, n_cu, GemvB13<true>::wpc(), p3v_tuning().gemv_wpw);
  out[0] = g.upw; out[1] = g.waves; out[2] = g.wpw; out[3] = p3v_cdiv(g.waves, g.wpw);
  return P3V_OK;
}

static int b13_launch_step(const GemvB13P& p, int K, bool scaled, bool begin, const GemvStepP& sp, hipStream_t s) {
  if (K == 8192) return begin ? launch_gemv_stream<GemvB13<false>, 1, 4, 4, STEP_BEGIN>(p, s, &sp) : launch_gemv_stream<GemvB13<false>, 1, 4, 4, STEP_END>(p, s, &sp);
  if (scaled) return begin ? launch_gemv_stream<GemvB13<true>, 1, 1, 6, STEP_BEGIN>(p, s, &sp) : launch_gemv_stream<GemvB13<true>, 1, 1, 6, STEP_END>(p, s, &sp);
  return begin ? launch_gemv_stream<GemvB13<false>, 1, 1, 6, STEP_BEGIN>(p, s, &sp) : launch_gemv_stream<GemvB13<false>, 1, 1, 6, STEP_END>(p, s, &sp);
}

extern "C" int p3v_gemv_b13_step(const p3v_gemv_b13_args_t* a, const p3v_gemv_step_t* st, void* stream) {
  if (!a || !st || !a->W || !a->out) return P3V_ERR_ARG;
  GemvStepP sp; bool begin, scaled;
  if (const int rc = gemv_step_params(a, st, true, sp, begin)) return rc;
  GemvB13P p;
  if (const int rc = b13_params(a, p, scaled)) return rc;
  hipStream_t s = (hipStream_t)stream;
  return b13_launch_step(p, a->K, scaled, begin, sp, s);
}

extern "C" int p3v_gemv_b13(const p3v_gemv_b13_args_t* a, void* stream) {
  if (!a || !a->x || !a->W || !a->out) return P3V_ERR_ARG;
  if (a->epilogue != P3V_EPI_NONE && a->epilogue != P3V_EPI_RESID_BF16 && a->epilogue != P3V_EPI_SILU_MUL &&
      a->epilogue != P3V_EPI_F32)
    return P3V_ERR_UNSUPPORTED;
  if (a->epilogue == P3V_EPI_RESID_BF16 && !a->resid) return P3V_ERR_ARG;
  GemvB13P p; bool scaled;
  if (const int rc = b13_params(a, p, scaled)) return rc;
  hipStream_t s = (hipStream_t)stream;
  if (a->K == 8192) return launch_gemv_stream<GemvB13<false>, 1, 4, 4>(p, s);
  return scaled ? launch_gemv_stream<GemvB13<true>, 1, 1, 6>(p, s) : launch_gemv_stream<GemvB13<false>, 1, 1, 6>(p, s);
}
```

### phi-3-vision-mlx_amd/csrc/p3v_runtime.hip

```cpp
#include <ctype.h>
#include <stdlib.h>
#include <string.h>

#include <mutex>

#include "p3v_common.h"

extern "C" int p3v_version(void) { return P3V_VERSION; }

extern "C" const char* p3v_strerror(int code) {
  switch (code) {
    case P3V_OK: return "ok";
    case P3V_ERR_ARG: return "invalid argument (shape, alignment or null pointer)";
    case P3V_ERR_LAUNCH: return "kernel launch failed";
    case P3V_ERR_UNSUPPORTED: return "unsupported combination";
    case P3V_ERR_HIP: return "HIP runtime call failed";
    default: return "unknown error";
  }
}

namespace {
struct Knob { const char* name; int P3vTuning::*field; int dflt; };
const Knob kKnobs[] = {
    {"gemm_big_rows", &P3vTuning::gemm_big_rows, -1},       {"gemm_no_splitk", &P3vTuning::gemm_no_splitk, 0},
    {"gemm_splitk_max_m", &P3vTuning::gemm_splitk_max_m, 1024}, {"gemm_splitk_max_s", &P3vTuning::gemm_splitk_max_s, 8},
    {"gemm_splitk_wgs", &P3vTuning::gemm_splitk_wgs, 256},  {"gemm_128", &P3vTuning::gemm_128, 0},
    {"gemm_persistent", &P3vTuning::gemm_persistent, 1},     {"gemm_no_qkv_fuse", &P3vTuning::gemm_no_qkv_fuse, 0},
    {"gemm_f8_narrow", &P3vTuning::gemm_f8_narrow, -1},     {"attn_no_dma", &P3vTuning::attn_no_dma, 0},
    {"attn_old", &P3vTuning::attn_old, 0},                  {"attn_pp", &P3vTuning::attn_pp, -1},
    {"attn_il", &P3vTuning::attn_il, -1},                   {"attn_il_waves", &P3vTuning::attn_il_waves, -1},
                      {"combine_g", &P3vTuning::combine_g, -1},
    {"kvq_old", &P3vTuning::kvq_old, 0},                    {"q8_old", &P3vTuning::q8_old, 0},
    {"gemv_no_mfma", &P3vTuning::gemv_no_mfma, 0},          {"gemv_no_mfma8", &P3vTuning::gemv_no_mfma8, 0},
    {"gemv_wpc", &P3vTuning::gemv_wpc, 8},                  {"gemv8_wgs", &P3vTuning::gemv8_wgs, 256},
    {"gemv_variant", &P3vTuning::gemv_variant, 3},          {"gemv_rows", &P3vTuning::gemv_rows, 1},
    {"gemv8_min", &P3vTuning::gemv8_min, 2},                {"gemv_mfma8", &P3vTuning::gemv_mfma8, 1},
    {"gemv_f8_wpc", &P3vTuning::gemv_f8_wpc, 16},           {"gemv_q4_wpc", &P3vTuning::gemv_q4_wpc, 8},
    {"gemv_wpw", &P3vTuning::gemv_wpw, 0},                  {"gemv_q4_rows_wgs", &P3vTuning::gemv_q4_rows_wgs, 256},
    {"gemv_q4_rows8", &P3vTuning::gemv_q4_rows8, 1},
    {"gemv_b13_wpc", &P3vTuning::gemv_b13_wpc, 16},         {"gemv_b13_wpc_end", &P3vTuning::gemv_b13_wpc_end, 8},
    {"gemv_b13_xscale", &P3vTuning::gemv_b13_xscale, 1},
    {"gemm_no_skinny", &P3vTuning::gemm_no_skinny, 0},     {"gemm_skinny_max_m", &P3vTuning::gemm_skinny_max_m, 256},
    {"gemm_skinny_s", &P3vTuning::gemm_skinny_s, 0},            {"gemm_skinny_tm128", &P3vTuning::gemm_skinny_tm128, 0},
    {"gemm_rows", &P3vTuning::gemm_rows, 1},
    {"attn_fo_map", &P3vTuning::attn_fo_map, 2},              {"attn_fo_map_q8", &P3vTuning::attn_fo_map_q8, 0},
};
P3vTuning g_tuning;
std::once_flag g_tuning_once;
void tuning_init() {
  for (const Knob& k : kKnobs) {
    char env[64] = "P3V_";
    size_t n = 4;
    for (const char* c = k.name; *c && n + 1 < sizeof(env); ++c) env[n++] = (char)toupper((unsigned char)*c);
    env[n] = 0;
    const char* e = getenv(env);
    g_tuning.*(k.field) = !e ? k.dflt : !strcmp(e, "auto") ? -1 : (*e == 0 ? 1 : atoi(e));
  }
}
}

const P3vTuning& p3v_tuning() {
  std::call_once(g_tuning_once, tuning_init);
  return g_tuning;
}

extern "C" int p3v_set_tuning(const char* name, int value) {
  if (!name) return P3V_ERR_ARG;
  std::call_once(g_tuning_once, tuning_init);
  for (const Knob& k : kKnobs)
    if (!strcmp(k.name, name)) { g_tuning.*(k.field) = value; return P3V_OK; }
  return P3V_ERR_ARG;
}

extern "C" int p3v_get_tuning(const char* name, int* value) {
  if (!name || !value) return P3V_ERR_ARG;
  std::call_once(g_tuning_once, tuning_init);
  for (const Knob& k : kKnobs)
    if (!strcmp(k.name, name)) { *value = g_tuning.*(k.field); return P3V_OK; }
  return P3V_ERR_ARG;
}

extern "C" int p3v_device_props(int device, p3v_props_t* out) {
  if (!out) return P3V_ERR_ARG;
  hipDeviceProp_t pr;
  if (hipGetDeviceProperties(&pr, device) != hipSuccess) return P3V_ERR_HIP;
  memset(out, 0, sizeof(*out));
  out->cu_count = pr.multiProcessorCount;
  out->lds_per_cu = (int)pr.maxSharedMemoryPerMultiProcessor;
  out->wave_size = pr.warpSize;
  out->clock_khz = pr.clockRate;
  out->mem_clock_khz = pr.memoryClockRate;
  out->mem_bus_bits = pr.memoryBusWidth;
  out->hbm_bytes = (int64_t)pr.totalGlobalMem;
  strncpy(out->arch, pr.gcnArchName, sizeof(out->arch) - 1);
  return P3V_OK;
}

extern "C" int p3v_graph_begin(void* stream) {
  return hipStreamBeginCapture((hipStream_t)stream, hipStreamCaptureModeThreadLocal) == hipSuccess ? P3V_OK : P3V_ERR_HIP;
}

extern "C" int p3v_graph_end(void* stream, void** graph_exec_out) {
  if (!graph_exec_out) return P3V_ERR_ARG;
  hipGraph_t g = nullptr;
  if (hipStreamEndCapture((hipStream_t)stream, &g) != hipSuccess || !g) return P3V_ERR_HIP;
  hipGraphExec_t ge = nullptr;
  const hipError_t e = hipGraphInstantiate(&ge, g, nullptr, nullptr, 0);
  (void)hipGraphDestroy(g);
  if (e != hipSuccess) return P3V_ERR_HIP;
  *graph_exec_out = (void*)ge;
  return P3V_OK;
}

extern "C" int p3v_graph_launch(void* graph_exec, void* stream) {
  if (!graph_exec) return P3V_ERR_ARG;
  return hipGraphLaunch((hipGraphExec_t)graph_exec, (hipStream_t)stream) == hipSuccess ? P3V_OK : P3V_ERR_HIP;
}

extern "C" int p3v_graph_destroy(void* graph_exec) {
  if (!graph_exec) return P3V_OK;
  return hipGraphExecDestroy((hipGraphExec_t)graph_exec) == hipSuccess ? P3V_OK : P3V_ERR_HIP;
}

extern "C" int p3v_event_create(void** ev) {
// ... 18 lines not shown
```

### phi-3-vision-mlx_amd/model.py

```python
import math
import copy
import os

import numpy as np
import torch

from . import ops, steps
from .parallel import families_without, family_pays, family_table
from .config import head_dim, is_vision, rope_scaling_factor
from .weights import Q4Weight, mlx_quantize, q4_repack
from .ops import (BF16, EPI_BIAS, EPI_BIAS_GELU, EPI_BIAS_QGELU, EPI_BIAS_RESID_F32, EPI_NONE, EPI_PATCH,
                  EPI_RESID_BF16, EPI_SILU_MUL, F32, I32)

import functools
import weakref


def _on_device(fn):
    @functools.wraps(fn)
    def wrapped(self, *a, **kw):
        with torch.cuda.device(self.device):
            return fn(self, *a, **kw)
    return wrapped

# ... 78 lines not shown
        view.sin = self.sin[rows]
        view.pad_len = self.pad_len[rows]
        if self.quantized:
            view.k8 = self.k8[:, rows]
            view.v8 = self.v8[:, rows]
            view.ks = self.ks[:, rows]
            view.vs = self.vs[:, rows]
            view.k_tmp = self.k_tmp[rows]
            view.v_tmp = self.v_tmp[rows]
        else:
            view.k = self.k[:, rows]
            view.v = self.v[:, rows]
        return view

    def mark_dirty(self):
        self.shared["dirty"] = True

    def scrub(self, lo, hi):
        hi = min(hi, self.Tp)
        if hi <= lo:
            return
        if self.quantized:
            self.v8[..., lo:hi] = 128
            self.k8[:, :, :, lo:hi] = 128
            self.vs[..., lo:hi] = 1.0
            self.ks[..., lo:hi] = 1.0
        else:
            self.v[..., lo:hi] = 0
            self.k[:, :, :, lo:hi] = 0


class LayerCache:

    def __init__(self, state, i):
        self.state, self.i = state, i

    @property
    def offset(self):
        return self.state.offset

    @offset.setter
    def offset(self, v):
        self.state.offset = int(v)


@steps.methods(_on_device)
class Phi3VModel:
    def __init__(self, cfg, weights, device="cuda:0"):
        if not torch.cuda.is_available():
            raise RuntimeError("Phi3VModel needs a GPU: the hot path is HIP-only (no CPU fallback)")
        ops.L.lib()
        self.cfg, self.device = cfg, torch.device(device)
        self.vision = is_vision(cfg)
        self.w = {k: v.to(self.device, BF16).contiguous() for k, v in weights.items() if not isinstance(v, Q4Weight)}
        self.w4 = {k: tuple(t.to(self.device) for t in q4_repack(*v)) for k, v in weights.items() if isinstance(v, Q4Weight)}
        self.hd = head_dim(cfg)
        if self.hd != 96:
            raise ValueError(f"decoder head_dim must be 96 (got {self.hd})")
        self.hidden_hook = None
        self.w8 = {}
        self._rope_tables = {}
        self._vit_graphs, self._vit_seen = {}, {}
        self.adapters = {}
        self._lora_tmp = {}
        self._lora_flat = None
        self.adapter_names = []
        self._bank = {}
        self._bank_keep = []
        self._rows_cur = None
        self.serving = os.environ.get("P3V_SHARED_GPU", "0") == "1"
        self.epoch = 0
        self._prefill_graphs = {}
        self._prefill_seen = {}
        self._states = weakref.WeakSet()
        self.fp8_act = bool(getattr(cfg, "fp8_activations", True)) and os.environ.get("P3V_FP8_PREFILL", "mfma") != "dequant"
        if getattr(cfg, "quantized_fp8", False):
            self._quantize_decoder_fp8()
        if getattr(cfg, "quantized_int4", False):
            self._quantize_decoder_q4()
        if self.w4 and not hasattr(self, "_deq"):
            n_max = max(v[0].shape[0] * v[0].shape[1] * 8 for v in self.w4.values())
            self._deq = torch.empty(n_max, dtype=BF16, device=self.device)
        self.w13 = {}
        if os.environ.get("P3V_PACK13", "1") != "0":
            self._pack_decoder_b13()
        if self.vision:
            self._prep_vision()

    def _quantize_decoder_fp8(self):
        names = [k for k in self.w if k == "lm_head.weight" or (k.startswith("model.layers.") and k.endswith("_proj.weight"))]
        for k in names:
            self.w8[k] = ops.quantize_fp8_rows(self.w.pop(k))
        n_max = max(v[0].shape[0] * v[0].shape[1] for v in self.w8.values())
        self._deq = torch.empty(n_max, dtype=BF16, device=self.device)

    @_on_device
    def _pack_decoder_b13(self):
        for k, v in self.w.items():
            if k != "lm_head.weight" and not (k.startswith("model.layers.") and k.endswith(("qkv_proj.weight", "gate_up_proj.weight", "down_proj.weight"))):
                continue
            if v.dim() != 2 or v.shape[1] not in (3072, 8192) or v.shape[0] % 2:
                continue
            pk = ops.pack_b13(v, silu_pairs=k.endswith("gate_up_proj.weight"))
            if pk is not None:
                self.w13[k] = pk

    def _packed(self, key):
        pk = self.w13.get(key)
        if pk is not None and not pk.current(self.w.get(key)):
            del self.w13[key]
            self.epoch += 1
            return None
        return pk

    def repack_b13(self):
        self.w13.clear()
        self.epoch += 1
        for st in list(self._states):
            st.graphs.clear()
        if os.environ.get("P3V_PACK13", "1") != "0":
            self._pack_decoder_b13()

    def set_adapters(self, adapters):
        if adapters and self._bank:
            raise ValueError("this model carries an adapter bank (set_adapter_bank): detach it before set_adapters -- one or the other")
        self._set_adapters(adapters)

    @_on_device
    def _set_adapters(self, adapters):
        for k, (a, b, _) in adapters.items():
            shape = self._weight_shape(k)
            if tuple(a.shape[:1]) != (shape[1],) or tuple(b.shape[1:]) != (shape[0],):
                raise ValueError(f"LoRA shapes {tuple(a.shape)} x {tuple(b.shape)} do not fit {k} {tuple(shape)}")
        self.adapters = {k: (a.to(self.device, F32).contiguous(), b.to(self.device, F32).contiguous(), float(s))
                         for k, (a, b, s) in adapters.items()}
        self.epoch += 1
        for st in list(self._states):
            st.graphs.clear()
        self._lora_tmp, self._lora_flat = {}, None
        self._prefill_graphs.clear()

    def _weight_shape(self, k):
        if k in self.w:
            return tuple(self.w[k].shape)
        if k in self.w8:
            return tuple(self.w8[k][0].shape)
        return (self.w4[k][0].shape[0], self.w4[k][0].shape[1] * 8)

    def set_adapter_bank(self, bank):
        bank = dict(bank or {})
        if not bank and not self._bank:
            return
        if bank and self.adapters:
            raise ValueError("this model carries a set_adapters adapter: detach it (set_adapters({})) before set_adapter_bank -- one or the other")
        for name, ad in bank.items():
            if not isinstance(name, str) or not name:
                raise ValueError(f"adapter names are non-empty strings, got {name!r}")
            for k, (a, b, _) in ad.items():
                if not (k.startswith("model.layers.") and k.endswith("_proj.weight")) or not (k in self.w or k in self.w8 or k in self.w4):
                    raise ValueError(f"adapter {name!r}: {k} is not a decoder projection of this model")
                shape = self._weight_shape(k)
                if a.dim() != 2 or b.dim() != 2 or a.shape[0] != shape[1] or b.shape[1] != shape[0] or a.shape[1] != b.shape[0]:
                    raise ValueError(f"adapter {name!r}: LoRA shapes {tuple(a.shape)} x {tuple(b.shape)} do not fit {k} {tuple(shape)}")
                if not 1 <= a.shape[1] <= ops.L.LORA_MAX_RANK:
                    raise ValueError(f"adapter {name!r}: rank {a.shape[1]} of {k} is outside 1..{ops.L.LORA_MAX_RANK}")
        self._attach_bank(bank)

    @_on_device
    def _attach_bank(self, bank):
        names = list(bank)
        dev = {n: {k: (a.to(self.device, F32).contiguous(), b.to(self.device, F32).contiguous(), float(s)) for k, (a, b, s) in ad.items()}
               for n, ad in bank.items()}
        union = sorted({k for ad in dev.values() for k in ad})
        self._bank = {k: (ops.lora_table([dev[n].get(k) for n in names], self.device), max(dev[n][k][0].shape[1] for n in names if k in dev[n]))
                      for k in union}
        self._bank_keep, self.adapter_names = dev, names
        self.epoch += 1
        for st in list(self._states):
            st.graphs.clear()
        self._lora_tmp, self._lora_flat = {}, None
        self._prefill_graphs.clear()

    def _bank_has(self, suffix):
        return any(k.endswith(suffix) for k in self._bank)

    def _state_rows(self, st):
        if st.row_adapter is None:
            st.row_adapter = torch.full((st.B,), -1, dtype=I32, device=self.device)
        return st.row_adapter

    @_on_device
    def set_row_adapters(self, st, adapters, row0=0):
        if isinstance(adapters, (str, int)) or adapters is None:
            adapters = [adapters]
        slots = []
        for a in adapters:
            if a is None:
                slots.append(-1)
            elif isinstance(a, str):
                if a not in self.adapter_names:
# ... 558 lines not shown
        decode = L <= ops.L.DECODE_MAX_L
        if bufs is None:
            bufs = self._plan(st, B, L, fuse_o=decode and n_beam == 1, family=n_beam == 1)
        q, o, qkv, a, h, n_split, ws = (bufs[k] for k in ("q", "o", "qkv", "a", "h", "n_split", "ws"))
        fuse_o, attn_merge = bufs.get("fuse_o", False), bufs.get("attn_merge", False)
        if decode and d_past is not None:
            rc, rs, rb = bufs["rope_cos"], bufs["rope_sin"], L
        elif decode:
            rc, rs, rb = st.cos[:, past:], st.sin[:, past:], st.T
        if self._bank:
            ra = self._state_rows(st)
            self._rows_cur = ra if M == st.B else ra.repeat_interleave(M // st.B)
        mlx4 = st.mlx4
        if (st.quantized or mlx4) and n_beam > 1:
            raise NotImplementedError("Beam Search is not yet compatible with Quantized Cache")
        mlx4_first = mlx4 and past == 0 and st.mlx4_tokens == 0 and L <= st.k4.shape[3]
        if n_beam > 1:
            Lp = (L + 7) // 8 * 8
            k_new = torch.empty((B, nkv, Lp, hd), dtype=BF16, device=self.device)
            v_new = torch.zeros((B, nkv, hd, Lp), dtype=BF16, device=self.device)
        normed_in = False
        for i in range(cfg.num_hidden_layers):
            p = f"model.layers.{i}."
            fused_qkv = False
            k_w = p + "self_attn.qkv_proj.weight"
            if (not decode and n_beam == 1 and k_w in w and k_w not in self.adapters and k_w not in self._bank and not mlx4_first
                    and (M >= 1024 or M <= 256) and os.environ.get("P3V_QKV_FUSE", "1") != "0"):
                kd, vd = (st.k_tmp, st.v_tmp) if st.quantized else (st.k[i], st.v[i])
                if not (st.quantized and past > 0 and not st.fresh_rows):
                    hn = h if normed_in else ops.rmsnorm(x, w[p + "input_layernorm.weight"], eps, out=h)
                    normed_in = True
                    fused_qkv = ops.gemm_qkv(hn, w[k_w], st.cos, st.sin, q, kd, vd, B, L, nh, nkv, hd, past, st.Tp, True, st.T, 1,
                                             q_scale=scale * ops.Q_PRESCALE)
            if i == 0 and step_begin is not None:
                sb = step_begin
                w_fold = w.get(k_w) if k_w in w else (self.w8.get(k_w) or self.w4.get(k_w))
                if B == 1 and self._packed(k_w) is not None:
                    w_fold = self.w13[k_w]
                if not (w_fold is not None and k_w not in self.adapters and k_w not in self._bank and os.environ.get("P3V_STEP_FOLD", "1") != "0"
                        and ops.gemv_step_begin(sb["tok"], sb["table"], x, st.cos, st.sin, d_past, sb["cos_o"], sb["sin_o"],
                                                w_fold, w[p + "input_layernorm.weight"], eps, qkv)):
                    ops.step_begin(sb["tok"], sb["table"], x, st.cos, st.sin, d_past, sb["cos_o"], sb["sin_o"])
                    self._proj(x, k_w, norm_w=w[p + "input_layernorm.weight"], out=qkv, h=h)
            elif not fused_qkv:
                if normed_in:
                    self._proj(h, p + "self_attn.qkv_proj.weight", out=qkv)
                else:
                    self._proj(x, p + "self_attn.qkv_proj.weight", norm_w=w[p + "input_layernorm.weight"], out=qkv, h=h)
            o_i = o
            if fuse_o:
                o_i, o_other = (bufs["o_f"], bufs["o_f2"]) if i % 2 == 0 else (bufs["o_f2"], bufs["o_f"])
            if st.quantized:
                if decode:
                    kw_o = {}
                    if fuse_o:
                        w8o = self.w8[p + "self_attn.o_proj.weight"]
                        kw_o = dict(o_proj_w8=w8o[0], o_proj_scale=w8o[1], o_proj_x=x, o_rearm=o_other)
                    ops.attention_decode_q8(qkv, rc, rs, rb, st.k8[i], st.v8[i], st.ks[i], st.vs[i], o_i, B, L, nh, nkv,
                                            hd, scale, past, st.Tp, ws, n_split, pad_len=st.pad_len, d_past=d_past,
                                            merge_in_launch=attn_merge, **kw_o)
                else:
                    if past > 0 and not st.fresh_rows:
                        ops.kv_dequantize(st.k8[i], st.v8[i], st.ks[i], st.vs[i], st.k_tmp, st.v_tmp, past)
                    if not fused_qkv:
                        ops.rope_kv_append(qkv, st.cos, st.sin, q, st.k_tmp, st.v_tmp, B, L, nh, nkv, hd, past, st.Tp, True, st.T, 1,
                                           q_scale=scale * ops.Q_PRESCALE)
                    ops.attention(q, o, B, L, nh, nkv, hd, scale, True, past=past, k_past=st.k_tmp, v_past=st.v_tmp,
                                  past_t=st.Tp, pad_len=st.pad_len, new_is_cache=True, q_prescaled=True)
                    ops.kv_quantize(st.k_tmp, st.v_tmp, st.k8[i], st.v8[i], st.ks[i], st.vs[i], past, L)
            elif n_beam > 1:
                ops.rope_kv_append(qkv, st.cos, st.sin, q, k_new, v_new, B, L, nh, nkv, hd, past, Lp, False, st.T, n_beam)
                ops.attention(q, o, B, L, nh, nkv, hd, scale, True, k_new=k_new, v_new=v_new, new_t=Lp, past=past,
                              k_past=st.k[i], v_past=st.v[i], past_t=st.Tp, past_div=n_beam, pad_len=st.pad_len,
                              pad_div=n_beam, ws=ws, n_split=n_split)
            elif decode and bufs.get("family"):
                ops.attention_decode_family(qkv, rc, rs, rb, st.k[i], st.v[i], o_i, B, nh, nkv, hd, scale,
                                            past if d_past is None else bufs.get("past_lb", -1), st.Tp, ws, n_split, st.family,
                                            family_host=st.family_host, pad_len=st.pad_len, d_past=d_past)
            elif decode:
                kw_o = {}
                if fuse_o:
                    q4o = self.w4.get(p + "self_attn.o_proj.weight")
                    kw_o = dict(o_proj_w=q4o[0], o_proj_sb=q4o[1]) if q4o is not None else dict(o_proj_w=w[p + "self_attn.o_proj.weight"])
                    kw_o.update(o_proj_x=x, o_rearm=o_other)
                ops.attention_decode(qkv, rc, rs, rb, st.k[i], st.v[i], o_i, B, L, nh, nkv, hd, scale,
                                     past if d_past is None else bufs.get("past_lb", -1), st.Tp, ws, n_split,
                                     pad_len=st.pad_len, d_past=d_past, merge_in_launch=attn_merge, **kw_o)
            else:
                if not fused_qkv:
                    ops.rope_kv_append(qkv, st.cos, st.sin, q, st.k[i], st.v[i], B, L, nh, nkv, hd, past, st.Tp, True, st.T, 1,
                                       q_scale=scale * ops.Q_PRESCALE)
                ops.attention(q, o, B, L, nh, nkv, hd, scale, True, past=past, k_past=st.k[i], v_past=st.v[i],
                              past_t=st.Tp, pad_len=st.pad_len, new_is_cache=True, q_prescaled=True)
            if mlx4_first:
                self._mlx4_quantize(st, i, L, qkv, nh)
            if last_only and i == cfg.num_hidden_layers - 1 and L > 1:
                o = o.view(B, L, -1)[:, -1].contiguous()
                x = x.view(B, L, -1)[:, -1].contiguous()
                a, h = a[:B], h[:B]
                if self._bank:
                    self._rows_cur = self._state_rows(st) if B == st.B else self._state_rows(st).repeat_interleave(B // st.B)
            normed = False
            if not (fuse_o and decode and n_beam == 1):
                normed = self._proj_resid_norm(o, p + "self_attn.o_proj.weight", x, w[p + "post_attention_layernorm.weight"], h)
                if not normed:
                    self._proj(o, p + "self_attn.o_proj.weight", EPI_RESID_BF16, resid=x, out=x)
            if normed:
                self._proj(h, p + "mlp.gate_up_proj.weight", EPI_SILU_MUL, out=a)
            else:
                self._proj(x, p + "mlp.gate_up_proj.weight", EPI_SILU_MUL, norm_w=w[p + "post_attention_layernorm.weight"], out=a, h=h)
            normed_in = False
            if i + 1 < cfg.num_hidden_layers:
                normed_in = self._proj_resid_norm(a, p + "mlp.down_proj.weight", x, w[f"model.layers.{i + 1}.input_layernorm.weight"], h)
            if not normed_in:
                self._proj(a, p + "mlp.down_proj.weight", EPI_RESID_BF16, resid=x, out=x)
            if self.hidden_hook is not None:
                self.hidden_hook(i, x, B, x.shape[0] // B)
        if mlx4_first:
            st.mlx4_tokens = L
        return x

    def _mlx4_quantize(self, st, i, L, qkv, nh):
        if st.k4.shape[3] != L:
            nl, B, nkv, _, g, _ = st.k4.shape
            st.k4 = torch.zeros((nl, B, nkv, L, g, 4), dtype=I32, device=self.device)
            st.v4 = torch.zeros_like(st.k4)
            st.k_sb = torch.zeros((nl, B, nkv, L, g, 2), dtype=F32, device=self.device)
            st.v_sb = torch.zeros_like(st.k_sb)
        ops.kv_quantize_mlx4(st.k[i], st.v[i], st.k4[i], st.v4[i], st.k_sb[i], st.v_sb[i], L, qkv=qkv, cos_t=st.cos, sin_t=st.sin, nh=nh,
                             past=0, tab_t=st.T, tab_div=1)

    def _build_decode_graph(self, st):
        cfg, B, dev = self.cfg, st.B, self.device
        g = dict(tok=torch.zeros((B,), dtype=I32, device=dev), d_past=torch.zeros((1,), dtype=I32, device=dev),
                 d_step=torch.zeros((1,), dtype=I32, device=dev),
                 history=torch.zeros((B, max(1, st.max_tokens) + 1), dtype=I32).pin_memory(),
                 x=torch.empty((B, cfg.hidden_size), dtype=BF16, device=dev),
                 logits=torch.empty((B, cfg.vocab_size), dtype=BF16, device=dev),
                 next_tok=torch.zeros((B,), dtype=I32, device=dev), ticket=torch.zeros((1,), dtype=I32, device=dev))
        g["bufs"] = self._plan(st, B, 1, fuse_o=not st.slots, captured=True)
        g["amax_ws"] = torch.zeros((ops.L.GEMV_STEP_WS_BYTES // 4,), dtype=F32, device=dev)
        g["d_past"].fill_(st.offset)
        g["gemm_ws"] = {}
        g["graph"] = self._capture(lambda: self._decode_step(st, g), g["gemm_ws"])
        g["d_step"].zero_()
        return g

    def _decode_step(self, st, g, kind=steps.GREEDY):
        cfg, w, bufs, head = self.cfg, self.w, g["bufs"], "lm_head.weight"
        self._layers(g["x"], st, st.B, 1, 0, 1, bufs=bufs, d_past=g["d_past"],
                     step_begin=dict(tok=g["tok"], table=w["model.embed_tokens.weight"], cos_o=bufs["rope_cos"], sin_o=bufs["rope_sin"]))
        end = (g["next_tok"], g["tok"], g["history"], g["d_step"], g["d_past"], g["ticket"])
        if not kind.sampled:
            w_fold = w.get(head) if head in w else (self.w8.get(head) or self.w4.get(head))
            if st.B == 1 and self._packed(head) is not None:
                w_fold = self.w13[head]
            if (w_fold is not None and head not in self.adapters and os.environ.get("P3V_STEP_FOLD", "1") != "0"
                    and ops.gemv_step_end(g["x"], w_fold, w["model.norm.weight"], cfg.rms_norm_eps, g["logits"], *end, g["amax_ws"])):
                return self._logprobs_tail(st, g) if kind.logprobs else None
        self._proj(g["x"], head, norm_w=w["model.norm.weight"], out=g["logits"], h=bufs["h"])
        if kind.penalized:
            pen = st.penalty
            ops.penalize(g["logits"], pen["rows"], pen["seen"], pen["bias"], g["tok"], out=pen["adj"])
            if kind.guided:
                self._guide_mask(pen["adj"], st.guide, slice(0, st.B), g["tok"])
            ops.sample_step_end(pen["adj"], st.sample_rows, *end)
# ... 452 lines not shown
```

### phi-3-vision-mlx_amd/ops.py

```python
import contextlib
import ctypes as C
import weakref

import numpy as np
import torch

from . import _lib as L
from ._lib import (EPI_BIAS, EPI_BIAS_GELU, EPI_BIAS_QGELU, EPI_BIAS_RESID_F32, EPI_F32, EPI_NONE,
                   EPI_PATCH, EPI_RESID_BF16, EPI_SILU_MUL)

BF16, F32, I32 = torch.bfloat16, torch.float32, torch.int32


def _stream():
    return torch.cuda.current_stream().cuda_stream


def _p(t):
    return 0 if t is None else t.data_ptr()


def _chk(t, dtype, name):
    if not t.is_cuda:
        raise RuntimeError(f"{name}: expected a device tensor (the hot path has no CPU fallback)")
# ... 317 lines not shown
    scale = torch.empty((M,), dtype=F32, device=x.device) if scale is None else scale
    L.check(L.lib().p3v_quant_fp8_rows(_p(x), _p(norm_w), float(norm_eps), _p(out), _p(scale), M, K, _stream()), "quant_fp8_rows")
    return out, scale


def gemm_fp8(a8, a_scale, w8, w_scale, epilogue=EPI_NONE, resid=None, out=None):
    _chk(a8, torch.uint8, "a8"), _chk(w8, torch.uint8, "w8"), _chk(a_scale, F32, "a_scale"), _chk(w_scale, F32, "w_scale")
    M, K = a8.shape
    N = w8.shape[0] // 2 if epilogue == EPI_SILU_MUL else w8.shape[0]
    if w8.shape[1] != K:
        raise ValueError(f"gemm_fp8: K mismatch {a8.shape} x {w8.shape}")
    out = torch.empty((M, N), dtype=BF16, device=a8.device) if out is None else out
    args = L.GemmF8Args(_p(a8), _p(a_scale), _p(w8), _p(w_scale), _p(out), _p(resid), M, N, K, a8.stride(0), w8.stride(0), N, epilogue)
    L.check(L.lib().p3v_gemm_fp8(C.byref(args), _stream()), "gemm_fp8")
    return out


def gemm_fp8_ok(M, N_rows, K, epilogue):
    n = N_rows // 2 if epilogue == EPI_SILU_MUL else N_rows
    return K % 128 == 0 and n % (128 if epilogue == EPI_SILU_MUL else 256) == 0 and epilogue in (EPI_NONE, EPI_RESID_BF16, EPI_SILU_MUL)


def linear(x, w, epilogue=EPI_NONE, resid=None, out=None):
    if x.shape[0] <= GEMV_MAX_M and x.shape[1] % 512 == 0 or x.shape[0] <= 8 and epilogue in (EPI_NONE, EPI_RESID_BF16, EPI_SILU_MUL, EPI_F32):
        return gemv(x, w, epilogue, resid=resid, out=out)
    return gemm(x, w, epilogue, resid=resid, out=out)


def rope_table(pos, inv_freq, scale):
    _chk(pos, F32, "pos"), _chk(inv_freq, F32, "inv_freq")
    n, half = pos.numel(), inv_freq.numel()
    cos = torch.empty((n, half), dtype=F32, device=pos.device)
    sin = torch.empty_like(cos)
    L.check(L.lib().p3v_rope_table(_p(pos), _p(inv_freq), float(scale), _p(cos), _p(sin), n, half, _stream()), "rope_table")
    return cos, sin


def rope_kv_append(qkv, cos_t, sin_t, q_out, k_dst, v_dst, B, Lq, nh, nkv, hd, past, dst_t, dst_off_is_past, tab_t=0,
                   tab_div=1, d_past=None, q_scale=1.0):
    L.check(L.lib().p3v_rope_kv_append(_p(qkv), _p(cos_t), _p(sin_t), _p(q_out), _p(k_dst), _p(v_dst), B, Lq, nh, nkv, hd,
                                       int(past), _p(d_past), dst_t, int(dst_off_is_past), tab_t, tab_div, float(q_scale),
                                       _stream()),
            "rope_kv_append")


def gemm_qkv(a, w, cos_t, sin_t, q_out, k_dst, v_dst, B, Lq, nh, nkv, hd, past, dst_t, dst_off_is_past, tab_t=0, tab_div=1,
             q_scale=1.0, bias=None):
    _chk(a, BF16, "a"), _chk(w, BF16, "w")
    M, K = a.shape
    g = L.GemmArgs(_p(a), _p(w), 0, _p(bias), 0, 0, M, w.shape[0], K, a.stride(0), w.stride(0), w.shape[0],
                   EPI_BIAS if bias is not None else EPI_NONE, 0, 0, 0)
    sp = L.QkvSplit(_p(cos_t), _p(sin_t), _p(q_out), _p(k_dst), _p(v_dst), B, Lq, nh, nkv, hd, int(past), dst_t, int(dst_off_is_past),
                    tab_t, tab_div, float(q_scale))
    rc = L.lib().p3v_gemm_qkv(C.byref(g), C.byref(sp), _stream())
    if rc == L.ERR_UNSUPPORTED:
        return False
    L.check(rc, "gemm_qkv")
    return True


Q_PRESCALE = 1.4426950408889634


def attention(q, out, B, Lq, nh, nkv, hd, scale, causal, k_new=None, v_new=None, new_t=0, past=0, k_past=None, v_past=None,
              past_t=0, past_div=1, pad_len=None, pad_div=1, d_past=None, ws=None, n_split=0, new_is_cache=False,
              q_prescaled=False):
    args = L.AttnArgs(_p(q), _p(k_past), _p(v_past), _p(k_new), _p(v_new), _p(out), _p(pad_len), _p(d_past), _p(ws),
                      B, Lq, nh, nkv, hd, int(past), past_t, past_div, new_t, pad_div, int(causal), float(scale), n_split, int(new_is_cache),
                      int(bool(q_prescaled)))
    L.check(L.lib().p3v_attention(C.byref(args), _stream()), "attention")
    return out


def attention_decode_can_fuse_oproj(B, Lq, nh, hd, n_split, cache_t, o_n, merge_in_launch):
    return bool(L.lib().p3v_attention_decode_can_fuse_oproj(B, Lq, nh, hd, n_split, cache_t, o_n, int(bool(merge_in_launch))))


def attention_decode_q8_can_fuse_oproj(B, Lq, nh, hd, n_split, cache_t, o_n, merge_in_launch):
    return bool(L.lib().p3v_attention_decode_q8_can_fuse_oproj(B, Lq, nh, hd, n_split, cache_t, o_n, int(bool(merge_in_launch))))


def attention_decode(qkv, cos_new, sin_new, rope_bstride, k_cache, v_cache, out, B, Lq, nh, nkv, hd, scale, past, cache_t, ws,
                     n_split, pad_len=None, d_past=None, merge_in_launch=False, o_proj_w=None, o_proj_x=None, o_rearm=None,
                     o_proj_sb=None):
    if o_proj_w is not None:
        if o_proj_sb is not None:
            _chk(o_proj_w, I32, "o_proj_w"), _chk(o_proj_sb, I32, "o_proj_sb")
            if tuple(o_proj_w.shape) != (o_proj_sb.shape[0], nh * hd // 8) or o_proj_sb.shape[1] != nh * hd // 64:
                raise ValueError("fused o_proj (4-bit): o_proj_w is [o_n, K / 8], o_proj_sb [o_n, K / 64]")
        else:
            _chk(o_proj_w, BF16, "o_proj_w")
            if o_proj_w.dim() != 2 or o_proj_w.shape[1] != nh * hd:
                raise ValueError(f"fused o_proj: o_proj_w must be [o_n, {nh * hd}], got {tuple(o_proj_w.shape)}")
        _chk(o_proj_x, BF16, "o_proj_x"), _chk(o_rearm, BF16, "o_rearm")
        if out.numel() < nh * hd or o_rearm.numel() < nh * hd:
            raise ValueError("fused o_proj: out and o_rearm are [n_heads * hd] rows")
        if o_proj_x.numel() < o_proj_w.shape[0]:
            raise ValueError(f"fused o_proj: o_proj_x holds {o_proj_x.numel()} values, the projection writes {o_proj_w.shape[0]}")
    args = L.AttnDecArgs(_p(qkv), _p(cos_new), _p(sin_new), _p(k_cache), _p(v_cache), _p(out), _p(pad_len), _p(d_past), _p(ws),
                         B, Lq, nh, nkv, hd, int(past), cache_t, rope_bstride, n_split, float(scale), int(bool(merge_in_launch)),
                         _p(o_proj_w), _p(o_proj_x), _p(o_rearm), 0 if o_proj_w is None else o_proj_w.shape[0], _p(o_proj_sb))
    L.check(L.lib().p3v_attention_decode(C.byref(args), _stream()), "attention_decode")
    return out


def attention_family_chunk(cache_t, n_split):
    return (-(-cache_t // n_split) + 63) & ~63


def attention_decode_family(qkv, cos_new, sin_new, rope_bstride, k_cache, v_cache, out, B, nh, nkv, hd, scale, past, cache_t, ws,
                            n_split, family, family_host=None, pad_len=None, d_past=None, Lq=1, merge_in_launch=False, o_proj_w=None):
    _chk(family, I32, "family")
    if tuple(family.shape) != (B, L.FAMILY_INTS):
        raise ValueError(f"family table must be [{B}, {L.FAMILY_INTS}], got {tuple(family.shape)}")
    host = None
    if family_host is not None:
        if family_host.is_cuda or family_host.dtype != torch.int32 or not family_host.is_contiguous() or \
                tuple(family_host.shape) != (B, L.FAMILY_INTS):
            raise ValueError(f"family_host must be a contiguous CPU int32 [{B}, {L.FAMILY_INTS}] tensor")
        host = family_host.data_ptr()
    args = L.AttnDecArgs(_p(qkv), _p(cos_new), _p(sin_new), _p(k_cache), _p(v_cache), _p(out), _p(pad_len), _p(d_past), _p(ws),
                         B, Lq, nh, nkv, hd, int(past), cache_t, rope_bstride, n_split, float(scale), int(bool(merge_in_launch)),
                         _p(o_proj_w), None, None, 0, None)
    L.check(L.lib().p3v_attention_decode_family(C.byref(args), _p(family), host, _stream()), "attention_decode_family")
    return out


def kv_quantize(k, vt, k8, v8t, k_scale, v_scale, t0, n_tok):
    B, nkv, src_t, hd = k.shape
    L.check(L.lib().p3v_kv_quantize(_p(k), _p(vt), _p(k8), _p(v8t), _p(k_scale), _p(v_scale), B * nkv, hd, src_t,
                                    k8.shape[2], int(t0), int(n_tok), _stream()), "kv_quantize")


def kv_quantize_mlx4(k, vt, k4, v4, k_sb, v_sb, n_tok, qkv=None, cos_t=None, sin_t=None, nh=0, past=0, tab_t=0, tab_div=1):
    _chk(k, BF16, "k"), _chk(vt, BF16, "vt"), _chk(k4, I32, "k4"), _chk(v4, I32, "v4"), _chk(k_sb, F32, "k_sb"), _chk(v_sb, F32, "v_sb")
    B, nkv, T, hd = k.shape
    if tuple(vt.shape) != (B, nkv, hd, T) or tuple(k4.shape) != (B, nkv, n_tok, hd // 32, 4) or tuple(k_sb.shape) != (B, nkv, n_tok, hd // 32, 2) \
            or k4.shape != v4.shape or k_sb.shape != v_sb.shape:
        raise ValueError("kv_quantize_mlx4: shapes")
    if qkv is not None:
        _chk(qkv, BF16, "qkv"), _chk(cos_t, F32, "cos_t"), _chk(sin_t, F32, "sin_t")
        if tuple(qkv.shape) != (B * n_tok, (nh + 2 * nkv) * hd):
            raise ValueError("kv_quantize_mlx4: qkv must be the projection output of exactly the n_tok tokens being quantised")
    L.check(L.lib().p3v_kv_quantize_mlx4(_p(k), _p(vt), _p(k4), _p(v4), _p(k_sb), _p(v_sb), B * nkv, hd, T, int(n_tok), _p(qkv), _p(cos_t),
                                         _p(sin_t), nh, nkv, int(past), tab_t, tab_div, _stream()), "kv_quantize_mlx4")


def kv_dequantize(k8, v8t, k_scale, v_scale, k, vt, n_tok):
    B, nkv, src_t, hd = k8.shape
    L.check(L.lib().p3v_kv_dequantize(_p(k8), _p(v8t), _p(k_scale), _p(v_scale), _p(k), _p(vt), B * nkv, hd, src_t, k.shape[2],
                                      int(n_tok), _stream()), "kv_dequantize")


def kv_copy(jobs):
    jobs = list(jobs)
    if not 1 <= len(jobs) <= L.KV_COPY_MAX_JOBS:
        raise ValueError(f"kv_copy: 1..{L.KV_COPY_MAX_JOBS} jobs per launch, got {len(jobs)}")
    recs = (L.KvCopyJob * len(jobs))()
    geom = None
    for rec, (src, b_src, t0_src, dst, b_dst, t0_dst, n_tok) in zip(recs, jobs):
        if len(src) != len(dst) or len(src) not in (2, 4):
            raise ValueError("kv_copy: a cache is (k, vt) or (k8, v8t, k_scale, v_scale), the same kind on both sides")
        dt = src[0].dtype
        if dt not in (BF16, torch.uint8) or (dt == BF16) != (len(src) == 2):
            raise TypeError(f"kv_copy: bf16 (k, vt) or uint8 codes with scales, got {dt} with {len(src)} tensors")
        for side in (src, dst):
            _chk(side[0], dt, "k"), _chk(side[1], dt, "vt")
            nl, B, nkv, T, hd = side[0].shape
            if tuple(side[1].shape) != (nl, B, nkv, hd, T):
                raise ValueError("kv_copy: V^T must be [nl, B, nkv, hd, T] of its K [nl, B, nkv, T, hd]")
            for sc in side[2:]:
                _chk(sc, F32, "scale")
                if tuple(sc.shape) != (nl, B, nkv, T):
                    raise ValueError("kv_copy: scale rows must be [nl, B, nkv, T]")
            g = (nl, nkv, hd, dt)
            if geom is None:
                geom = g
            elif g != geom:
                raise ValueError("kv_copy: every cache of a launch has the same layers, heads, head size and element type")
        rec.k_src, rec.v_src, rec.k_dst, rec.v_dst = _p(src[0]), _p(src[1]), _p(dst[0]), _p(dst[1])
        if len(src) == 4:
            rec.ks_src, rec.vs_src, rec.ks_dst, rec.vs_dst = _p(src[2]), _p(src[3]), _p(dst[2]), _p(dst[3])
        rec.B_src, rec.b_src, rec.T_src, rec.t0_src = src[0].shape[1], int(b_src), src[0].shape[3], int(t0_src)
        rec.B_dst, rec.b_dst, rec.T_dst, rec.t0_dst = dst[0].shape[1], int(b_dst), dst[0].shape[3], int(t0_dst)
# ... 409 lines not shown
```

Measured before the change: 578.8 tokens/s.

## Fuse 13-bit packed o_proj weights into the attention-decode projection epilogue

Packs each decoder layer's o_proj matrix into the lossless 13-bit b13 format and teaches the fused attention-decode o_proj epilogue (both in-launch and combine forms) to decode those weights instead of reading full bf16. The goal is to cut HBM bytes streamed for o_proj during memory-bound decode. It adds a per-block x-range check that falls back to exact bf16 x with base-added weights when inputs don't fit the scaled path, plus extra register pressure that may lower occupancy in the fused kernel. It also clears prefill graphs when packs change.

```diff
diff --git a/include/p3v.h b/include/p3v.h
--- a/include/p3v.h
+++ b/include/p3v.h
@@ -156,6 +156,7 @@
   int merge_in_launch;
   const void* o_proj_w; uint16_t* o_proj_x; uint16_t* o_rearm; int o_n;
   const uint32_t* o_proj_sb;
+  const void* o_proj_b13; int o_proj_b13_base;
 } p3v_attn_decode_args_t;
 int p3v_attention_decode(const p3v_attn_decode_args_t* args , void* stream);
 int p3v_attention_decode_can_fuse_oproj(int B, int L, int n_heads, int hd, int n_split, int cache_t, int o_n, int merge_in_launch);
diff --git a/phi-3-vision-mlx_amd/_lib.py b/phi-3-vision-mlx_amd/_lib.py
--- a/phi-3-vision-mlx_amd/_lib.py
+++ b/phi-3-vision-mlx_amd/_lib.py
@@ -78,7 +78,8 @@
                 ("B", i32), ("L", i32), ("n_heads", i32), ("n_kv", i32), ("hd", i32), ("past", i32),
                 ("cache_t", i32), ("rope_bstride", i32), ("n_split", i32), ("scale", f32), ("merge_in_launch", i32),
                 ("o_proj_w", vp), ("o_proj_x", vp), ("o_rearm", vp), ("o_n", i32),
-                ("o_proj_sb", vp)]
+                ("o_proj_sb", vp),
+                ("o_proj_b13", vp), ("o_proj_b13_base", i32)]
 
 
 class AttnDecQ8Args(C.Structure):
diff --git a/phi-3-vision-mlx_amd/csrc/p3v_attention.hip b/phi-3-vision-mlx_amd/csrc/p3v_attention.hip
--- a/phi-3-vision-mlx_amd/csrc/p3v_attention.hip
+++ b/phi-3-vision-mlx_amd/csrc/p3v_attention.hip
@@ -5,6 +5,7 @@
 #include "p3v_dot_bf16.h"
 #include "p3v_dot_f8.h"
 #include "p3v_dot_q4.h"
+#include "p3v_dot_b13.h"
 
 struct AttnP {
   const bf16_t* q; const bf16_t* k_past; const bf16_t* v_past; const bf16_t* k_new; const bf16_t* v_new;
@@ -1585,12 +1586,12 @@
 #ifndef P3V_FO_SLEEP
 #define P3V_FO_SLEEP 4
 #endif
-enum { FO_NONE = 0, FO_BF16 = 1, FO_F8 = 2, FO_Q4 = 3 };
-struct FoP { const void* o_w; const void* o_scale; bf16_t* o_x; const bf16_t* out; int nh; };
+enum { FO_NONE = 0, FO_BF16 = 1, FO_F8 = 2, FO_Q4 = 3, FO_B13 = 4 };
+struct FoP { const void* o_w; const void* o_scale; bf16_t* o_x; const bf16_t* out; int nh; uint32_t cc; int xscale; };
 template <int KIND, int NU = 1>
 __device__ __forceinline__ void fo_project(const FoP f, const int o_wl, unsigned char* lds, const int o_wl2 = -1) {
-  constexpr bool F8 = KIND == FO_F8, Q4 = KIND == FO_Q4;
-  constexpr int HD = 96, NJ = KIND == FO_BF16 ? 6 : 3;
+  constexpr bool F8 = KIND == FO_F8, Q4 = KIND == FO_Q4, B13F = KIND == FO_B13;
+  constexpr int HD = 96, NJ = KIND == FO_BF16 || B13F ? 6 : 3;
   const int tid = threadIdx.x, lane = tid & 63, wave = __builtin_amdgcn_readfirstlane(tid >> 6);
   const int Kd = f.nh * HD;
   const size_t row_bytes = (size_t)Kd * (Q4 ? 1 : F8 ? 2 : 4) / 2;
@@ -1599,6 +1600,8 @@
   u32x4_t ow[NU][2][Q4 ? 1 : NJ];
   u32x2_t oq[NU][2][Q4 ? 3 : 1];
   uint32_t osb[NU][2][Q4 ? 3 : 1];
+  [[maybe_unused]] uint32_t bsg[NU][B13<6>::NS];
+  [[maybe_unused]] u32x4_t bnib[NU][3], blo[NU][6];
   uint32_t ores[NU];
   float osc[NU][2];
 #pragma unroll
@@ -1615,6 +1618,8 @@
         osb[k][0][j] = s0[j * 16];
         osb[k][1][j] = s0[Kd / 64 + j * 16];
       }
+    } else if constexpr (B13F) {
+      b13_load<6>((const uint32_t*)f.o_w + (size_t)o_u[k] * B13<6>::DWORDS, lane, bsg[k], bnib[k], blo[k]);
     } else {
 #pragma unroll
       for (int j = 0; j < NJ; ++j) {
@@ -1627,7 +1632,19 @@
     osc[k][1] = F8 ? ((const float*)f.o_scale)[2 * o_u[k] + 1] : 1.f;
   }
   {
+    if constexpr (B13F) {
+#pragma unroll
+      for (int k = 0; k < NU; ++k) {
+        if (k == 1 && !two) continue;
+#pragma unroll
+        for (int j = 0; j < 6; ++j)
+#pragma unroll
+          for (int h = 0; h < 2; ++h)
+            ow[k][h][j] = f.xscale ? b13_weights<false, 6>(bsg[k], bnib[k], blo[k], 0u, j, h) : b13_weights<true, 6>(bsg[k], bnib[k], blo[k], f.cc, j, h);
+      }
+    }
     __shared__ int o_timeout;
+    __shared__ int o_unfit[4];
     const uint32_t* src = (const uint32_t*)f.out;
     if (wave == 0) {
       bool to = false;
@@ -1644,9 +1661,10 @@
     __syncthreads();
     uint32_t* xs = (uint32_t*)lds;
     bool timeout = o_timeout != 0;
+    uint32_t xv[6];
+    const uint32_t cc_x = B13F && f.xscale ? f.cc : 0u;
     {
       const int NW = f.nh * HD / 2 / 4;
-      uint32_t xv[6];
       for (unsigned tries = 0; !timeout; ++tries) {
         bool bad = false;
 #pragma unroll
@@ -1657,12 +1675,38 @@
         if (tries >= (1u << 12)) timeout = true;
         __builtin_amdgcn_s_sleep(2);
       }
-#pragma unroll
-      for (int j = 0; j < 6; ++j) xs[wave * NW + j * 64 + lane] = xv[j];
+      if constexpr (B13F) {
+        uint32_t xacc[2] = {0u, 0xffffffffu};
+#pragma unroll
+        for (int j = 0; j < 6; ++j) xs[wave * NW + j * 64 + lane] = b13_stage_x(cc_x, xv[j], xacc);
+        const bool any = __builtin_amdgcn_ballot_w64(b13_x_unfit(cc_x, xacc)) != 0;
+        if (lane == 0) o_unfit[wave] = any;
+      } else {
+#pragma unroll
+        for (int j = 0; j < 6; ++j) xs[wave * NW + j * 64 + lane] = xv[j];
+      }
       if (timeout && lane == 0) o_timeout = 1;
     }
     __syncthreads();
     timeout = o_timeout != 0;
+    [[maybe_unused]] bool b13_exact = true;
+    if constexpr (B13F) {
+      b13_exact = !f.xscale || ((o_unfit[0] | o_unfit[1]) | (o_unfit[2] | o_unfit[3])) != 0;
+      if (f.xscale && b13_exact) {
+        const int NW = f.nh * HD / 2 / 4;
+#pragma unroll
+        for (int j = 0; j < 6; ++j) xs[wave * NW + j * 64 + lane] = xv[j];
+#pragma unroll
+        for (int k = 0; k < NU; ++k)
+#pragma unroll
+          for (int j = 0; j < 6; ++j)
+#pragma unroll
+            for (int h = 0; h < 2; ++h)
+#pragma unroll
+              for (int d = 0; d < 4; ++d) ow[k][h][j][d] = b13_add_base(ow[k][h][j][d], f.cc);
+        __syncthreads();
+      }
+    }
     float* xsum = (float*)(lds + 6144);
     if (Q4) {
       if (tid < 192) {
@@ -1726,7 +1770,8 @@
 
 template <int FO = 0>
 __device__ __forceinline__ void attn_decode_body128(const AttnDecP& p, const int bx, const int by, const int bz, unsigned char* KV,
-                                                    const int o_unit = -2, const int o_unit2 = -1) {
+                                                    const int o_unit = -2, const int o_unit2 = -1,
+                                                    const uint32_t o_cc = 0u, const int o_xscale = 0) {
   constexpr int TK = 128, WK = 32, HD = 96, KROW = HD * 2, VROWB = TK * 2, NKS = 3, NDT = 6, CPR = 12;
   constexpr int KS_BYTES = WK * KROW;
   static_assert(KS_BYTES >= 16 * HD * 4, "a wave's O partial reuses its K slice");
@@ -1983,7 +2028,7 @@
     split_merge<256>(p.ws + ((size_t)b * p.nh + head) * p.n_split * 16 * (HD + 2), p.out + (size_t)b * p.L * (p.nh * HD) + head * HD,
                      (size_t)p.nh * HD, p.L, p.n_split, own, (float*)vtile, FO != 0);
   if (FO && o_worker) {
-    fo_project<FO, 2>(FoP{p.o_w, p.o_sb, p.o_x, p.out, p.nh}, o_wl, KV, o_unit2);
+    fo_project<FO, 2>(FoP{p.o_w, p.o_sb, p.o_x, p.out, p.nh, o_cc, o_xscale}, o_wl, KV, o_unit2);
   }
 }
 
@@ -2010,6 +2055,16 @@
     bx = m.bx, by = m.by, o_unit = m.o_unit, o_unit2 = m.o_unit2;
   }
   attn_decode_body128<FO_Q4>(p, bx, by, blockIdx.z, KV, o_unit, o_unit2);
+}
+
+__global__ void __launch_bounds__(256) k_attn_decode128_o13(AttnDecP p, uint32_t cc, int xscale) {
+  __shared__ __attribute__((aligned(1024))) unsigned char KV[4 * 6144 + 96 * 256];
+  int bx = blockIdx.x, by = blockIdx.y, o_unit = -2, o_unit2 = -1;
+  if (p.fo_remap) {
+    const FoMap m = fo_map((int)blockIdx.x, p.n_split, p.nh, p.o_n / 8, p.fo_remap == 2);
+    bx = m.bx, by = m.by, o_unit = m.o_unit, o_unit2 = m.o_unit2;
+  }
+  attn_decode_body128<FO_B13>(p, bx, by, blockIdx.z, KV, o_unit, o_unit2, cc, xscale);
 }
 
 __global__ void __launch_bounds__(256) k_attn_decode(AttnDecP p) {
@@ -2267,6 +2322,21 @@
   const int n_uw = (int)gridDim.x - nh, u = (int)blockIdx.x - nh;
   fo_project<KIND, 2>(FoP{o_w, o_sb, o_x, out, nh}, u, lds, u + n_uw < n_units ? u + n_uw : -1);
 }
+__global__ void __launch_bounds__(512) k_attn_combine_o13(const float* __restrict__ ws, bf16_t* __restrict__ out, bf16_t* __restrict__ o_rearm,
+                                                          const void* o_w, bf16_t* o_x, int nh, int n_split, int n_units, uint32_t cc, int xscale) {
+  __shared__ __attribute__((aligned(16))) unsigned char lds[7 * 1024 + 768];
+  if ((int)blockIdx.x < nh) {
+    if (blockIdx.x == 0) {
+      uint32_t* ra = (uint32_t*)o_rearm;
+      for (int i = threadIdx.x; i < nh * 96 / 2; i += blockDim.x) ra[i] = 0xffffffffu;
+    }
+    combine_rows<true>(ws, out, 1, nh, 96, n_split, (int)blockIdx.x);
+    return;
+  }
+  if (threadIdx.x >= 256) return;
+  const int n_uw = (int)gridDim.x - nh, u = (int)blockIdx.x - nh;
+  fo_project<FO_B13, 2>(FoP{o_w, nullptr, o_x, out, nh, cc, xscale}, u, lds, u + n_uw < n_units ? u + n_uw : -1);
+}
 
 static bool combine_o_ok(int B, int L, int n_heads, int hd, int n_split, int o_n) {
   if (B != 1 || L != 1 || hd != 96 || n_heads * hd != 3072 || o_n <= 0 || o_n % 8) return false;
@@ -2285,6 +2355,14 @@
   P3V_CHECK_LAUNCH();
   return P3V_OK;
 }
+static int launch_combine_o13(const float* ws, void* out, void* o_rearm, const void* o_w13, uint32_t cc, int xscale, void* o_x, int n_heads,
+                              int n_split, int o_n, hipStream_t s) {
+  const int n_units = o_n / 8, grid_o = n_heads + (n_units + 1) / 2;
+  hipLaunchKernelGGL(k_attn_combine_o13, dim3(grid_o), dim3(combine_threads(n_split)), 0, s, ws, (bf16_t*)out, (bf16_t*)o_rearm, o_w13,
+                     (bf16_t*)o_x, n_heads, n_split, n_units, cc, xscale);
+  P3V_CHECK_LAUNCH();
+  return P3V_OK;
+}
 
 __global__ void k_stage_rope(const float* __restrict__ cos_t, const float* __restrict__ sin_t, const int32_t* d_past,
                              int past, float* __restrict__ cos_o, float* __restrict__ sin_o, int L, int tab_t, int half) {
@@ -2311,28 +2389,28 @@
 }
 #endif
 
+static long fo_capacity(int form) {
+  static long capacity_of[P3V_MAX_DEVICES][3] = {};
+  int dev = 0;
+  if (hipGetDevice(&dev) != hipSuccess || dev < 0 || dev >= P3V_MAX_DEVICES) return 0;
+  if (!capacity_of[dev][form]) {
+    int per_cu = 0;
+    hipDeviceProp_t pr;
+    if (hipGetDeviceProperties(&pr, dev) != hipSuccess) return 0;
+    const void* k = form == 0 ? (const void*)k_attn_decode128_o : form == 1 ? (const void*)k_attn_decode128_o4 : (const void*)k_attn_decode128_o13;
+    if (hipOccupancyMaxActiveBlocksPerMultiprocessor(&per_cu, k, 256, 0) != hipSuccess || per_cu < 1) return 0;
+    capacity_of[dev][form] = (long)per_cu * (pr.multiProcessorCount - 8);
+  }
+  return capacity_of[dev][form];
+}
+
 extern "C" int p3v_attention_decode_can_fuse_oproj(int B, int L, int n_heads, int hd, int n_split, int cache_t, int o_n, int merge_in_launch) {
   if (B != 1 || L != 1 || hd != 96 || n_heads * hd != 3072 || o_n <= 0 || o_n % 8) return 0;
   if (!merge_in_launch)
     return combine_o_ok(B, L, n_heads, hd, n_split, o_n) ? 2 : 0;
   if (!(n_split * 128 >= cache_t && cache_t % 128 == 0 && n_split * 64 < cache_t) || n_split < 2) return 0;
   if ((long)(n_split - 1) * n_heads * 8 < o_n) return 0;
-  static long capacity_of[P3V_MAX_DEVICES] = {0};
-  int dev = 0;
-  if (hipGetDevice(&dev) != hipSuccess || dev < 0 || dev >= P3V_MAX_DEVICES) return 0;
-  if (!capacity_of[dev]) {
-    int per_cu = 0;
-    hipDeviceProp_t pr;
-    if (hipGetDeviceProperties(&pr, dev) != hipSuccess) return 0;
-    int per_cu4 = 0;
-    if (hipOccupancyMaxActiveBlocksPerMultiprocessor(&per_cu, k_attn_decode128_o, 256, 0) != hipSuccess ||
-        hipOccupancyMaxActiveBlocksPerMultiprocessor(&per_cu4, k_attn_decode128_o4, 256, 0) != hipSuccess) return 0;
-    per_cu = min(per_cu, per_cu4);
-    if (per_cu < 1) return 0;
-    capacity_of[dev] = (long)per_cu * (pr.multiProcessorCount - 8);
-  }
-  const long capacity = capacity_of[dev];
-  return (long)B * n_heads * n_split <= capacity;
+  return (long)B * n_heads * n_split <= min(fo_capacity(0), fo_capacity(1));
 }
 
 extern "C" int p3v_attention_decode_fused_role(int wg, int n_heads, int n_split, int o_n, int map, int* out4) {
@@ -2357,17 +2435,28 @@
                 a->o_proj_w, a->o_proj_sb, (bf16_t*)a->o_proj_x, (bf16_t*)a->o_rearm, a->o_n, 0};
   hipStream_t s = (hipStream_t)stream;
   dim3 grid(a->n_split, a->n_heads, a->B);
+  if (a->o_proj_b13) {
+    if (!a->o_proj_w || a->o_proj_sb || ((uintptr_t)a->o_proj_b13 & 15) || a->o_proj_b13_base < 1 || a->o_proj_b13_base > 224) return P3V_ERR_ARG;
+    if (a->o_n != 3072 || a->n_heads * a->hd != 3072) return P3V_ERR_UNSUPPORTED;
+  }
   const int fuse_form = a->o_proj_w ? p3v_attention_decode_can_fuse_oproj(a->B, a->L, a->n_heads, a->hd, a->n_split, a->cache_t, a->o_n, a->merge_in_launch) : 0;
   if (a->o_proj_w && !fuse_form) return P3V_ERR_UNSUPPORTED;
   if (a->o_proj_w && (!a->o_proj_x || !a->o_rearm || ((uintptr_t)a->o_proj_w | (uintptr_t)a->o_proj_x | (uintptr_t)a->o_rearm) & 15)) return P3V_ERR_ARG;
   if (a->o_proj_w && a->o_proj_sb && ((uintptr_t)a->o_proj_sb & 3)) return P3V_ERR_ARG;
+  const int fo13 = p3v_tuning().attn_fo_b13;
+  const bool b13 = a->o_proj_b13 && ((fuse_form == 2 && fo13 >= 2) ||
+                                     (fuse_form == 1 && fo13 >= 1 && (long)a->B * a->n_heads * a->n_split <= fo_capacity(2)));
+  const uint32_t o_cc = b13 ? b13_cc(a->o_proj_b13_base) : 0u;
+  const int o_xscale = b13 && p3v_tuning().gemv_b13_xscale != 0 && a->o_proj_b13_base - 1 <= B13_XSCALE_MAX_SHIFT;
   if (fuse_form == 1) {
     if (p3v_tuning().attn_fo_map && fo_map_ok(a->n_split, a->n_heads, a->o_n)) {
       p.fo_remap = p3v_tuning().attn_fo_map;
       grid = dim3(a->n_split * a->n_heads, 1, 1);
     }
-    if (a->o_proj_sb) {
-      if ((uintptr_t)a->o_proj_sb & 3) return P3V_ERR_ARG;
+    if (b13) {
+      p.o_w = a->o_proj_b13;
+      hipLaunchKernelGGL(k_attn_decode128_o13, grid, dim3(256), 0, s, p, o_cc, o_xscale);
+    } else if (a->o_proj_sb) {
       hipLaunchKernelGGL(k_attn_decode128_o4, grid, dim3(256), 0, s, p);
     } else {
       hipLaunchKernelGGL(k_attn_decode128_o, grid, dim3(256), 0, s, p);
@@ -2380,6 +2469,8 @@
   else hipLaunchKernelGGL(k_attn_decode_stream<64>, grid, dim3(64), 0, s, p);
   P3V_CHECK_LAUNCH();
   if (a->merge_in_launch) return P3V_OK;
+  if (fuse_form == 2 && b13)
+    return launch_combine_o13(a->ws, a->out, a->o_rearm, a->o_proj_b13, o_cc, o_xscale, a->o_proj_x, a->n_heads, a->n_split, a->o_n, s);
   if (fuse_form == 2)
     return a->o_proj_sb ? launch_combine_o<FO_Q4>(a->ws, a->out, a->o_rearm, a->o_proj_w, a->o_proj_sb, a->o_proj_x, a->n_heads, a->n_split, a->o_n, s)
                         : launch_combine_o<FO_BF16>(a->ws, a->out, a->o_rearm, a->o_proj_w, nullptr, a->o_proj_x, a->n_heads, a->n_split, a->o_n, s);
diff --git a/phi-3-vision-mlx_amd/csrc/p3v_common.h b/phi-3-vision-mlx_amd/csrc/p3v_common.h
--- a/phi-3-vision-mlx_amd/csrc/p3v_common.h
+++ b/phi-3-vision-mlx_amd/csrc/p3v_common.h
@@ -133,5 +133,6 @@
   int gemv_no_mfma, gemv_no_mfma8, gemv_wpc, gemv8_wgs, gemv_variant, gemv_rows, gemv8_min, gemv_mfma8, gemv_f8_wpc, gemv_q4_wpc, gemv_wpw, gemv_q4_rows_wgs, gemv_q4_rows8;
   int gemv_b13_wpc, gemv_b13_wpc_end;
   int gemv_b13_xscale;
+  int attn_fo_b13;
 };
 const P3vTuning& p3v_tuning();
diff --git a/phi-3-vision-mlx_amd/csrc/p3v_dot_b13.h b/phi-3-vision-mlx_amd/csrc/p3v_dot_b13.h
--- a/phi-3-vision-mlx_amd/csrc/p3v_dot_b13.h
+++ b/phi-3-vision-mlx_amd/csrc/p3v_dot_b13.h
@@ -19,18 +19,75 @@
   pre[3] = __builtin_amdgcn_perm(hi1, lo1, 0x07030602u);
 }
 
+__device__ __forceinline__ uint32_t b13_add_base(uint32_t pre, uint32_t cc) {
+  const b13_u16x2_t c2 = __builtin_bit_cast(b13_u16x2_t, cc), one = {1, 1}, mag = {0x7fff, 0x7fff};
+  const b13_u16x2_t p = __builtin_bit_cast(b13_u16x2_t, pre);
+  b13_u16x2_t n, r;
+  asm("v_pk_min_u16 %0, %1, %2" : "=v"(n) : "v"(p & mag), "v"(one));
+  asm("v_pk_mad_u16 %0, %1, %2, %3" : "=v"(r) : "v"(n), "v"(c2), "v"(p));
+  return __builtin_bit_cast(uint32_t, r);
+}
+
 __device__ __forceinline__ u32x4_t b13_decode8(uint32_t lo0, uint32_t lo1, uint32_t nib, uint32_t sg0, uint32_t sg1, uint32_t cc) {
   uint32_t pre[4];
   b13_pre8(lo0, lo1, nib, sg0, sg1, pre);
-  const b13_u16x2_t c2 = __builtin_bit_cast(b13_u16x2_t, cc), one = {1, 1}, mag = {0x7fff, 0x7fff};
   u32x4_t w;
 #pragma unroll
-  for (int d = 0; d < 4; ++d) {
-    const b13_u16x2_t p = __builtin_bit_cast(b13_u16x2_t, pre[d]);
-    b13_u16x2_t n, r;
-    asm("v_pk_min_u16 %0, %1, %2" : "=v"(n) : "v"(p & mag), "v"(one));
-    asm("v_pk_mad_u16 %0, %1, %2, %3" : "=v"(r) : "v"(n), "v"(c2), "v"(p));
-    w[d] = __builtin_bit_cast(uint32_t, r);
-  }
+  for (int d = 0; d < 4; ++d) w[d] = b13_add_base(pre[d], cc);
   return w;
 }
+
+template <int CH>
+__device__ __forceinline__ void b13_load(const uint32_t* cp, int lane, uint32_t (&sg)[B13<CH>::NS], u32x4_t (&nib)[CH / 2], u32x4_t (&lo)[CH]) {
+  typedef B13<CH> L;
+  if constexpr (L::NS == 3) {
+    const uint32_t* sp = cp + lane * 3;
+    sg[0] = __builtin_nontemporal_load(sp);
+    sg[1] = __builtin_nontemporal_load(sp + 1);
+    sg[2] = __builtin_nontemporal_load(sp + 2);
+  } else {
+    const u32x2_t v = __builtin_nontemporal_load((const u32x2_t*)cp + lane);
+    sg[0] = v[0];
+    sg[1] = v[1];
+  }
+  const u32x4_t* np = (const u32x4_t*)(cp + L::NIB_OFF) + lane;
+  const u32x4_t* lp = (const u32x4_t*)(cp + L::LO_OFF) + lane;
+#pragma unroll
+  for (int i = 0; i < CH / 2; ++i) nib[i] = __builtin_nontemporal_load(np + i * 64);
+#pragma unroll
+  for (int j = 0; j < CH; ++j) lo[j] = __builtin_nontemporal_load(lp + j * 64);
+}
+
+template <bool EXACT, int CH>
+__device__ __forceinline__ u32x4_t b13_weights(const uint32_t (&sg)[B13<CH>::NS], const u32x4_t (&nibs)[CH / 2], const u32x4_t (&los)[CH], uint32_t cc,
+                                               int j, int row) {
+  typedef B13<CH> L;
+  const uint32_t lo0 = los[j][2 * row], lo1 = los[j][2 * row + 1], nib = nibs[j >> 1][(j & 1) * 2 + row];
+  const uint32_t sg0 = sg[L::sign_word(row, j, 0)] << L::sign_shift(row, j, 0), sg1 = sg[L::sign_word(row, j, 1)] << L::sign_shift(row, j, 1);
+  if constexpr (EXACT) return b13_decode8(lo0, lo1, nib, sg0, sg1, cc);
+  else {
+    uint32_t pre[4];
+    b13_pre8(lo0, lo1, nib, sg0, sg1, pre);
+    return (u32x4_t){pre[0], pre[1], pre[2], pre[3]};
+  }
+}
+
+#define B13_XSCALE_MAX_SHIFT 96
+static inline uint32_t b13_cc(int base) { const uint32_t c = (uint32_t)(base - 1) << 7; return c | (c << 16); }
+
+__device__ __forceinline__ uint32_t b13_stage_x(uint32_t cc, uint32_t x2, uint32_t (&acc)[2]) {
+  const b13_u16x2_t one = {1, 1};
+  const uint32_t mag = x2 & 0x7fff7fffu;
+  uint32_t nz, y2, m1;
+  asm("v_pk_min_u16 %0, %1, %2" : "=v"(nz) : "v"(mag), "v"(one));
+  asm("v_pk_mad_u16 %0, %1, %2, %3" : "=v"(y2) : "v"(nz), "v"(cc), "v"(x2));
+  asm("v_pk_max_u16 %0, %1, %2" : "=v"(acc[0]) : "v"(acc[0]), "v"(mag));
+  asm("v_pk_sub_u16 %0, %1, %2" : "=v"(m1) : "v"(mag), "v"(one));
+  asm("v_pk_min_u16 %0, %1, %2" : "=v"(acc[1]) : "v"(acc[1]), "v"(m1));
+  return y2;
+}
+__device__ __forceinline__ bool b13_x_unfit(uint32_t cc, const uint32_t (&acc)[2]) {
+  const uint32_t top = 0x7f80u - (cc & 0xffffu);
+  const uint32_t mx = max(acc[0] & 0xffffu, acc[0] >> 16), mn = min(acc[1] & 0xffffu, acc[1] >> 16);
+  return mx >= top || mn < 0x7fu;
+}
diff --git a/phi-3-vision-mlx_amd/csrc/p3v_gemv_b13.hip b/phi-3-vision-mlx_amd/csrc/p3v_gemv_b13.hip
--- a/phi-3-vision-mlx_amd/csrc/p3v_gemv_b13.hip
+++ b/phi-3-vision-mlx_amd/csrc/p3v_gemv_b13.hip
@@ -33,39 +33,14 @@
   static __device__ __forceinline__ void mark(int k) { B13MARK(k); }
   template <int K, int CH>
   static __device__ __forceinline__ void load(const P& p, int r0, int, int c0, Stage<CH>& st) {
-    typedef B13<CH> L;
     constexpr int NST = K / (CH * 512);
     const int u = p.epi == P3V_EPI_SILU_MUL ? r0 : r0 >> 1, lane = c0 & 63, s = (c0 >> 6) / CH;
-    const uint32_t* cp = p.W + (size_t)(u * NST + s) * L::DWORDS;
-    if constexpr (L::NS == 3) {
-      const uint32_t* sp = cp + lane * 3;
-      st.sg[0] = __builtin_nontemporal_load(sp);
-      st.sg[1] = __builtin_nontemporal_load(sp + 1);
-      st.sg[2] = __builtin_nontemporal_load(sp + 2);
-    } else {
-      const u32x2_t v = __builtin_nontemporal_load((const u32x2_t*)cp + lane);
-      st.sg[0] = v[0];
-      st.sg[1] = v[1];
-    }
-    const u32x4_t* np = (const u32x4_t*)(cp + L::NIB_OFF) + lane;
-    const u32x4_t* lp = (const u32x4_t*)(cp + L::LO_OFF) + lane;
-#pragma unroll
-    for (int i = 0; i < CH / 2; ++i) st.nib[i] = __builtin_nontemporal_load(np + i * 64);
-#pragma unroll
-    for (int j = 0; j < CH; ++j) st.lo[j] = __builtin_nontemporal_load(lp + j * 64);
+    b13_load<CH>(p.W + (size_t)(u * NST + s) * B13<CH>::DWORDS, lane, st.sg, st.nib, st.lo);
     if constexpr (!SCALED) st.cc = p.cc;
   }
   template <bool EXACT, int CH>
   static __device__ __forceinline__ u32x4_t weights_as(const Stage<CH>& st, uint32_t cc, int j, int row) {
-    typedef B13<CH> L;
-    const uint32_t lo0 = st.lo[j][2 * row], lo1 = st.lo[j][2 * row + 1], nib = st.nib[j >> 1][(j & 1) * 2 + row];
-    const uint32_t sg0 = st.sg[L::sign_word(row, j, 0)] << L::sign_shift(row, j, 0), sg1 = st.sg[L::sign_word(row, j, 1)] << L::sign_shift(row, j, 1);
-    if constexpr (EXACT) return b13_decode8(lo0, lo1, nib, sg0, sg1, cc);
-    else {
-      uint32_t pre[4];
-      b13_pre8(lo0, lo1, nib, sg0, sg1, pre);
-      return (u32x4_t){pre[0], pre[1], pre[2], pre[3]};
-    }
+    return b13_weights<EXACT, CH>(st.sg, st.nib, st.lo, cc, j, row);
   }
   template <int CH>
   static __device__ __forceinline__ u32x4_t weights(const Stage<CH>& st, int j, int row) {
@@ -89,22 +64,8 @@
     a0 = dot8(weights_as<true>(st, p.cc, j, 0), xa, a0);
     a1 = dot8(weights_as<true>(st, p.cc, j, 1), xa, a1);
   }
-  static __device__ __forceinline__ uint32_t stage_x(const P& p, uint32_t x2, uint32_t (&acc)[2]) {
-    const b13_u16x2_t one = {1, 1};
-    const uint32_t mag = x2 & 0x7fff7fffu;
-    uint32_t nz, y2, m1;
-    asm("v_pk_min_u16 %0, %1, %2" : "=v"(nz) : "v"(mag), "v"(one));
-    asm("v_pk_mad_u16 %0, %1, %2, %3" : "=v"(y2) : "v"(nz), "v"(p.cc), "v"(x2));
-    asm("v_pk_max_u16 %0, %1, %2" : "=v"(acc[0]) : "v"(acc[0]), "v"(mag));
-    asm("v_pk_sub_u16 %0, %1, %2" : "=v"(m1) : "v"(mag), "v"(one));
-    asm("v_pk_min_u16 %0, %1, %2" : "=v"(acc[1]) : "v"(acc[1]), "v"(m1));
-    return y2;
-  }
-  static __device__ __forceinline__ bool x_unfit(const P& p, const uint32_t (&acc)[2]) {
-    const uint32_t top = 0x7f80u - (p.cc & 0xffffu);
-    const uint32_t mx = max(acc[0] & 0xffffu, acc[0] >> 16), mn = min(acc[1] & 0xffffu, acc[1] >> 16);
-    return mx >= top || mn < 0x7fu;
-  }
+  static __device__ __forceinline__ uint32_t stage_x(const P& p, uint32_t x2, uint32_t (&acc)[2]) { return b13_stage_x(p.cc, x2, acc); }
+  static __device__ __forceinline__ bool x_unfit(const P& p, const uint32_t (&acc)[2]) { return b13_x_unfit(p.cc, acc); }
   template <int CH> static __device__ __forceinline__ float finish(float v, const Stage<CH>&, int) { return v; }
 };
 
@@ -200,7 +161,6 @@
 }
 
 static bool b13_shape_ok(int rows, int K) { return rows > 0 && rows % 2 == 0 && (K == 3072 || K == 8192); }
-static uint32_t b13_cc(int base) { const uint32_t c = (uint32_t)(base - 1) << 7; return c | (c << 16); }
 
 extern "C" int p3v_pack_b13(const uint16_t* W, int rows, int K, int silu_pairs, void* out, int32_t* info, void* stream) {
   if (!W || !out || !info) return P3V_ERR_ARG;
@@ -229,7 +189,6 @@
   return P3V_OK;
 }
 
-#define B13_XSCALE_MAX_SHIFT 96
 static int b13_params(const p3v_gemv_b13_args_t* a, GemvB13P& p, bool& scaled) {
   if (a->M <= 0 || a->N <= 0) return P3V_ERR_ARG;
   if (a->M != 1 || a->N % 2 || (a->K != 3072 && a->K != 8192)) return P3V_ERR_UNSUPPORTED;
diff --git a/phi-3-vision-mlx_amd/csrc/p3v_runtime.hip b/phi-3-vision-mlx_amd/csrc/p3v_runtime.hip
--- a/phi-3-vision-mlx_amd/csrc/p3v_runtime.hip
+++ b/phi-3-vision-mlx_amd/csrc/p3v_runtime.hip
@@ -39,7 +39,7 @@
     {"gemv_wpw", &P3vTuning::gemv_wpw, 0},                  {"gemv_q4_rows_wgs", &P3vTuning::gemv_q4_rows_wgs, 256},
     {"gemv_q4_rows8", &P3vTuning::gemv_q4_rows8, 1},
     {"gemv_b13_wpc", &P3vTuning::gemv_b13_wpc, 16},         {"gemv_b13_wpc_end", &P3vTuning::gemv_b13_wpc_end, 8},
-    {"gemv_b13_xscale", &P3vTuning::gemv_b13_xscale, 1},
+    {"gemv_b13_xscale", &P3vTuning::gemv_b13_xscale, 1},   {"attn_fo_b13", &P3vTuning::attn_fo_b13, 1},
     {"gemm_no_skinny", &P3vTuning::gemm_no_skinny, 0},     {"gemm_skinny_max_m", &P3vTuning::gemm_skinny_max_m, 256},
     {"gemm_skinny_s", &P3vTuning::gemm_skinny_s, 0},            {"gemm_skinny_tm128", &P3vTuning::gemm_skinny_tm128, 0},
     {"gemm_rows", &P3vTuning::gemm_rows, 1},
diff --git a/phi-3-vision-mlx_amd/model.py b/phi-3-vision-mlx_amd/model.py
--- a/phi-3-vision-mlx_amd/model.py
+++ b/phi-3-vision-mlx_amd/model.py
@@ -184,6 +184,7 @@
             n_max = max(v[0].shape[0] * v[0].shape[1] * 8 for v in self.w4.values())
             self._deq = torch.empty(n_max, dtype=BF16, device=self.device)
         self.w13 = {}
+        self.w13o = {}
         if os.environ.get("P3V_PACK13", "1") != "0":
             self._pack_decoder_b13()
         if self.vision:
@@ -199,25 +200,31 @@
     @_on_device
     def _pack_decoder_b13(self):
         for k, v in self.w.items():
-            if k != "lm_head.weight" and not (k.startswith("model.layers.") and k.endswith(("qkv_proj.weight", "gate_up_proj.weight", "down_proj.weight"))):
+            o_proj = k.startswith("model.layers.") and k.endswith("self_attn.o_proj.weight")
+            if k != "lm_head.weight" and not o_proj and not (
+                    k.startswith("model.layers.") and k.endswith(("qkv_proj.weight", "gate_up_proj.weight", "down_proj.weight"))):
                 continue
             if v.dim() != 2 or v.shape[1] not in (3072, 8192) or v.shape[0] % 2:
                 continue
             pk = ops.pack_b13(v, silu_pairs=k.endswith("gate_up_proj.weight"))
             if pk is not None:
-                self.w13[k] = pk
+                (self.w13o if o_proj else self.w13)[k] = pk
 
     def _packed(self, key):
-        pk = self.w13.get(key)
+        held = self.w13 if key in self.w13 else self.w13o
+        pk = held.get(key)
         if pk is not None and not pk.current(self.w.get(key)):
-            del self.w13[key]
+            del held[key]
             self.epoch += 1
+            self._prefill_graphs.clear()
             return None
         return pk
 
     def repack_b13(self):
         self.w13.clear()
+        self.w13o.clear()
         self.epoch += 1
+        self._prefill_graphs.clear()
         for st in list(self._states):
             st.graphs.clear()
         if os.environ.get("P3V_PACK13", "1") != "0":
@@ -942,6 +949,8 @@
                 if fuse_o:
                     q4o = self.w4.get(p + "self_attn.o_proj.weight")
                     kw_o = dict(o_proj_w=q4o[0], o_proj_sb=q4o[1]) if q4o is not None else dict(o_proj_w=w[p + "self_attn.o_proj.weight"])
+                    if q4o is None:
+                        kw_o.update(o_proj_b13=self._packed(p + "self_attn.o_proj.weight"))
                     kw_o.update(o_proj_x=x, o_rearm=o_other)
                 ops.attention_decode(qkv, rc, rs, rb, st.k[i], st.v[i], o_i, B, L, nh, nkv, hd, scale,
                                      past if d_past is None else bufs.get("past_lb", -1), st.Tp, ws, n_split,
diff --git a/phi-3-vision-mlx_amd/ops.py b/phi-3-vision-mlx_amd/ops.py
--- a/phi-3-vision-mlx_amd/ops.py
+++ b/phi-3-vision-mlx_amd/ops.py
@@ -423,7 +423,15 @@
 
 def attention_decode(qkv, cos_new, sin_new, rope_bstride, k_cache, v_cache, out, B, Lq, nh, nkv, hd, scale, past, cache_t, ws,
                      n_split, pad_len=None, d_past=None, merge_in_launch=False, o_proj_w=None, o_proj_x=None, o_rearm=None,
-                     o_proj_sb=None):
+                     o_proj_sb=None, o_proj_b13=None):
+    if o_proj_b13 is not None:
+        if o_proj_w is None or o_proj_sb is not None:
+            raise ValueError("fused o_proj (13-bit): o_proj_b13 goes with the bf16 o_proj_w it was packed from")
+        if o_proj_b13.silu_pairs:
+            raise ValueError("fused o_proj (13-bit): the matrix must be packed by neighbouring rows (silu_pairs=False)")
+        if o_proj_b13.rows != o_proj_w.shape[0] or o_proj_b13.K != nh * hd or o_proj_b13.K != 3072:
+            raise ValueError(f"fused o_proj (13-bit): packed [{o_proj_b13.rows}, {o_proj_b13.K}] does not match o_proj_w "
+                             f"{tuple(o_proj_w.shape)} with K = n_heads * hd = 3072")
     if o_proj_w is not None:
         if o_proj_sb is not None:
             _chk(o_proj_w, I32, "o_proj_w"), _chk(o_proj_sb, I32, "o_proj_sb")
@@ -440,7 +448,8 @@
             raise ValueError(f"fused o_proj: o_proj_x holds {o_proj_x.numel()} values, the projection writes {o_proj_w.shape[0]}")
     args = L.AttnDecArgs(_p(qkv), _p(cos_new), _p(sin_new), _p(k_cache), _p(v_cache), _p(out), _p(pad_len), _p(d_past), _p(ws),
                          B, Lq, nh, nkv, hd, int(past), cache_t, rope_bstride, n_split, float(scale), int(bool(merge_in_launch)),
-                         _p(o_proj_w), _p(o_proj_x), _p(o_rearm), 0 if o_proj_w is None else o_proj_w.shape[0], _p(o_proj_sb))
+                         _p(o_proj_w), _p(o_proj_x), _p(o_rearm), 0 if o_proj_w is None else o_proj_w.shape[0], _p(o_proj_sb),
+                         None if o_proj_b13 is None else _p(o_proj_b13.data), 0 if o_proj_b13 is None else o_proj_b13.base)
     L.check(L.lib().p3v_attention_decode(C.byref(args), _stream()), "attention_decode")
     return out
 
```

New measurement: 573.6 tokens/s. Within noise of the previous version (-0.9%).
